# z3lx/waifu2x-tensorrt

Hardware: AMD Instinct MI355X
Metric: upscaled MPix/s, 1080p->4K swin_unet/art fp16 (higher is better)
Workload: dtype f16; 1 GPU; configs[2]: swin_unet/art scale4 noise3 batch4 tile256 fp16, 1920x1080 frame, blend=0.0625 (45 tiles, 12 batches); synthetic-weight graph of that architecture, frame resident in HBM; frames_per_rank=132, parallelism=frame-sharded x1, no collectives; timing barrier over gloo, mode=frames, tiles_per_network_pass=48, tile_groups_per_pass=2

## Files before the change

### waifu2x-tensorrt_amd/csrc/engine.cpp

```cpp
#include <hip/hip_runtime.h>
#include <dlfcn.h>

#include <algorithm>
#include <array>
#include <chrono>
#include <cmath>
#include <cstdio>
#include <cstdlib>
#include <cstring>
#include <deque>
#include <filesystem>
#include <fstream>
#include <map>
#include <sstream>
#include <tuple>

#include "../../include/w2x/img2img.h"
#include "common.h"
#include "fragorder.h"
#include "kernels.h"
#include "liveness.h"
#include "lower.h"
#include "plan.h"
#include "schedule.h"
// ... 133 lines not shown

}

struct Img2Img::Impl {
    MessageCallback messageCallback{};
    ProgressCallback progressCallback{};

    void log(Severity s, const std::string& m) { if (messageCallback) messageCallback(s, m); }
    void log(Severity s, const std::string& m, const std::string& fn, int line) { if (messageCallback) messageCallback(s, "[" + fn + "@" + std::to_string(line) + "] " + m); }
    void log(int current, int total, double speed) { Impl* const to = report_to ? report_to : this; if (to->progressCallback) to->progressCallback(current, total, speed); }
    Impl* report_to = nullptr;

    bool loaded = false;
    int device = -1;
    bool poison = false;
    bool check_general = false;
    bool use_graphs = true;
    Plan plan;
    RenderConfig cfg;
    hipStream_t stream = nullptr;
    hipEvent_t ev0 = nullptr, ev1 = nullptr;
    int (*roctx_push)(const char*) = nullptr; int (*roctx_pop)() = nullptr;
    hipEvent_t ev_shard = nullptr;
    hipEvent_t ev_part[kMaxRenderParts] = {nullptr, nullptr, nullptr, nullptr};
    int pipeline_parts = 3;
    size_t shard_halo_slots = 0;
    int shard_rows = 0, shard_cols = 0;
    hipStream_t gstream[3] = {nullptr, nullptr, nullptr};
    hipEvent_t ev_fork = nullptr, ev_join[3] = {nullptr, nullptr, nullptr};
    int groups = 2;
    std::vector<void*> tensors, blobs;
    std::vector<void*> frag_blobs;
    std::vector<void*> perm_blobs;
    std::vector<int> pool_blocks;
    void* arena_base = nullptr; size_t arena_bytes = 0;
    std::vector<GemmParams> gemm;
    int final_op = -1;
    std::vector<Launch> launches;
    std::vector<std::array<void*, 4>> launch_planes;

    bool deep = false;
    uint8_t* d_frame = nullptr; size_t frame_cap = 0;
    uint8_t* d_out = nullptr; size_t out_cap = 0;
    void* d_slab = nullptr; size_t slab_cap = 0;
    void* d_slab2 = nullptr; size_t slab2_cap = 0;
    hipEvent_t ev_g0[2] = {nullptr, nullptr}, ev_cmp[2] = {nullptr, nullptr};
    bool rolling = false;
    bool rolling_ok = true;
    TileSlot* d_slots = nullptr; size_t slots_cap = 0;
    LiveExt* d_live = nullptr; size_t live_cap = 0, live_stride = 0;
    std::vector<LiveExt> h_live;
    std::map<std::pair<int, int>, std::vector<OpExtent>> live_cache;
    void upload_live(const TileGrid& grid, size_t count, hipStream_t on) {
        const size_t nops = plan.ops.size();
        if (!count || !nops) return;
        if (count > live_stride) {
            ensure(d_live, live_cap, (nops * count + 8) * sizeof(LiveExt));
            live_stride = count;
        }
        const bool all = switches().no_dead_skip || check_general || cfg.tta;
        std::map<std::pair<int, int>, int> tile_at;
        if (!all) for (int t = 0; t < grid.count; ++t) tile_at[{grid.in[t].x, grid.in[t].y}] = t;
        auto extents = [&](int w, int h) -> const std::vector<OpExtent>& {
            auto it = live_cache.find({w, h});
            if (it == live_cache.end()) it = live_cache.emplace(std::make_pair(w, h), dead_skip_extents(plan, w, h, false)).first;
            return it->second;
        };
        const std::vector<OpExtent>& whole = extents(plan.Tout, plan.Tout);
        h_live.resize(nops * count);
        for (size_t st = 0; st < count; ++st) {
            const TileSlot& sl = h_slots[st];
            const std::vector<OpExtent>* e = &whole;
            if (!all && sl.valid && sl.aug == 0) {
                const auto it = tile_at.find({sl.x, sl.y});
                if (it != tile_at.end()) e = &extents(grid.out[it->second].w, grid.out[it->second].h);
            }
            for (size_t i = 0; i < nops; ++i) {
                const OpExtent& x = (*e)[i];
                auto u16 = [](int v) { return (uint16_t)std::min(std::max(v, 0), 65535); };
                h_live[i * count + st] = x.all() ? LiveExt{65535, 0, 65535, 0} : LiveExt{u16(x.x.c), u16(x.x.w), u16(x.y.c), u16(x.y.w)};
            }
        }
        hipAssert(hipMemcpy2DAsync(d_live, live_stride * sizeof(LiveExt), h_live.data(), count * sizeof(LiveExt), count * sizeof(LiveExt), nops, hipMemcpyHostToDevice, on));
    }
    float *d_rampx = nullptr, *d_rampy = nullptr;
    int ovx = 0, ovy = 0;
    float* d_blob_in = nullptr; float* d_blob_out = nullptr;
    uint8_t* d_frame2 = nullptr; size_t frame2_cap = 0;
    uint8_t* d_out2 = nullptr; size_t out2_cap = 0;
    hipStream_t s_up = nullptr, s_dn = nullptr;
    hipEvent_t ev_up[2] = {nullptr, nullptr}, ev_comp[2] = {nullptr, nullptr}, ev_dn[2] = {nullptr, nullptr};
    float* d_canvas = nullptr; size_t canvas_cap = 0;
    struct ResizeTables {
        int inW = 0, inH = 0, outW = 0, outH = 0, filter = 0, edge = kEdgeReplicate;
        int *fx = nullptr, *fy = nullptr; float *wx = nullptr, *wy = nullptr;
        int kx = 0, ky = 0, rows_max = 0;
        int rows_max_above = 0;
    };
    std::deque<ResizeTables> rs_tables;
    struct YuvJob { YuvCoefs in, out; int in_bits = 8, out_bits = 8, key = 0, in_layout = kYuvI420, out_layout = kYuvI420, in_siting = kYuvLeft, out_siting = kYuvLeft; };
    uint8_t* d_bgr = nullptr; size_t bgr_cap = 0;
    uint8_t* d_alpha = nullptr; size_t alpha_cap = 0;
    unsigned* d_minmax = nullptr; unsigned* h_minmax = nullptr;
    hipEvent_t ev_minmax = nullptr;
    struct RgbaJob { int bleed = 0; bool skip = false; size_t alpha_slot0 = 0; bool uniform = false; unsigned value = 255; };
    struct GrayJob { bool deep = false; };
    struct PlanarJob { int in_bits = 8, out_bits = 8; };
    struct ChainJob { const void* src = nullptr; void* dst = nullptr; bool dst_fp32 = false; };
    struct Job {
        enum Kind { BGR, YUV, RGBA, GRAY, PLANAR, PLANAR_RGBA } kind = BGR;
        const ResizeTables* rs = nullptr;
        YuvJob yuv;
        RgbaJob rgba;
        GrayJob gray;
        PlanarJob planar;
        ChainJob chain;
    };
    DitherOptions dither;
    unsigned seq_frame = 0;
    const uint16_t* d_noise = nullptr;
    DitherArgs dither_now() {
        const int mode = (int)dither.mode;
        if (mode == kDitherNone) return DitherArgs();
        if (mode == kDitherBlueNoise && !d_noise) {
            hipError_t e = hipSuccess;
            d_noise = dither_table_device(&e);
            hipAssert(e);
        }
        return dither_args(mode, dither.phase + seq_frame * dither.advance, mode == kDitherBlueNoise ? d_noise : nullptr);
    }
    ResizeLight light = ResizeLight::Gamma;
    LightArgs light_now() const { return light_args((int)light); }
    int edge = kEdgeReplicate;
    bool edge_refuses(const char* who, const char* what) {
        if (edge == kEdgeReplicate) return false;
        log(Severity::error, std::string(what) + " not built under setEdge(" + edge_mode_name(edge) + "): only setEdge(replicate) serves this call.", who, __LINE__);
        return true;
    }
    Job job;
    struct JobScope { Impl* im; ~JobScope() { im->job = Job{}; } };
    static constexpr int kChainStages = 4;
    void* d_chain[kChainStages - 1] = {nullptr, nullptr, nullptr}; size_t chain_cap[kChainStages - 1] = {0, 0, 0};
    hipEvent_t ev_chain_done[kChainStages] = {nullptr, nullptr, nullptr, nullptr}, ev_chain_read[kChainStages - 1] = {nullptr, nullptr, nullptr};
    struct StageTables { TileSlot* d_slots = nullptr; size_t slots_cap = 0; LiveExt* d_live = nullptr; size_t live_cap = 0, live_stride = 0; std::vector<LiveExt> h_live; std::vector<TileSlot> h_slots; };
    StageTables chain_tables[kChainStages];
    void swap_tables(int k) {
        StageTables& t = chain_tables[k];
        std::swap(d_slots, t.d_slots); std::swap(slots_cap, t.slots_cap); std::swap(d_live, t.d_live); std::swap(live_cap, t.live_cap); std::swap(live_stride, t.live_stride);
        h_live.swap(t.h_live); h_slots.swap(t.h_slots);
    }
    void ensure_chain(int k, size_t bytes) {
        if (bytes <= chain_cap[k]) return;
        if (d_chain[k]) hipAssert(hipFree(d_chain[k]));
        d_chain[k] = nullptr; chain_cap[k] = 0;
        hipAssert(hipMalloc(&d_chain[k], bytes));
        chain_cap[k] = bytes;
    }
    std::vector<void*> pinned;
    std::vector<void*> host_allocs;
    std::vector<TileSlot> h_slots;

    bool profiling = false;
    struct Stamp { int kind; hipEvent_t a, b; double flops; int op; };
    std::vector<double> op_ms;
    std::vector<Stamp> stamps;
    void stamp_begin(int kind, double flops, int op = -1) {
        if (!profiling) return;
        Stamp st{kind, nullptr, nullptr, flops, op};
        hipAssert(hipEventCreate(&st.a)); hipAssert(hipEventCreate(&st.b));
        hipAssert(hipEventRecord(st.a, stream));
        stamps.push_back(st);
    }
    void stamp_end() { if (profiling) hipAssert(hipEventRecord(stamps.back().b, stream)); }

    void ensure_copy_streams() {
        if (s_up) return;
        hipAssert(hipStreamCreateWithFlags(&s_up, hipStreamNonBlocking));
        hipAssert(hipStreamCreateWithFlags(&s_dn, hipStreamNonBlocking));
        for (int b = 0; b < 2; ++b) { hipAssert(hipEventCreateWithFlags(&ev_up[b], hipEventDisableTiming)); hipAssert(hipEventCreateWithFlags(&ev_comp[b], hipEventDisableTiming)); hipAssert(hipEventCreateWithFlags(&ev_dn[b], hipEventDisableTiming)); }
    }

    bool one_part_stale = false;
    void one_part_slots() {
        if (!one_part_stale) return;
        const size_t stepCount = pass_slots(last_strip.tile_count);
        fill_slots(last_grid, last_strip.first_tile, last_strip.tile_count, 1, 0, stepCount);
        upload_slots(last_grid, stepCount, stepCount);
        hipAssert(hipStreamSynchronize(stream));
        one_part_stale = false;
    }
    int batch_count(int tiles) const { return w2x::batch_count(tiles, cfg.tta ? 8 : 1, plan.userB); }
    size_t pass_slots(int tiles) const { return w2x::pass_slots(tiles, cfg.tta ? 8 : 1, plan.userB, plan.B); }
    void fill_slots(const TileGrid& grid, int first, int tiles, int valid, size_t at, size_t count) {
        const int steps = cfg.tta ? 8 : 1;
        if (h_slots.size() < at + count) h_slots.resize(at + count);
        for (size_t st = 0; st < count; ++st) {
            const int ti = (int)(st / steps), aug = (int)(st % steps);
            TileSlot sl{0, 0, aug, 0};
            if (ti < tiles) { sl.x = grid.in[first + ti].x; sl.y = grid.in[first + ti].y; sl.valid = valid; }
            h_slots[at + st] = sl;
        }
    }
    void upload_slots(const TileGrid& grid, size_t count, size_t slab_slots) {
        ensure(d_slots, slots_cap, count * sizeof(TileSlot));
        hipAssert(hipMemcpyAsync(d_slots, h_slots.data(), count * sizeof(TileSlot), hipMemcpyHostToDevice, stream));
        upload_live(grid, count, stream);
        ensure(d_slab, slab_cap, slab_slots * plan.Tout * plan.Tout * 4 * plan.elt);
    }
    int last_rows = 0, last_cols = 0, last_batches = 0;
    TileGrid last_grid;
    StripPlan last_strip;
    float last_ms = 0.f;

    static constexpr int kRgbaKey = 64;
    static constexpr int kGrayKey = 65;
    static constexpr int kPlanarKey = 67;
    static constexpr int kPlanarRgbaKey = 72;
    static constexpr int kChainKey = 80;
    using GraphKey = std::tuple<const void*, const void*, const void*, const void*, int, int, int, int>;
    struct PassGraphs { hipGraphExec_t g[4] = {nullptr, nullptr, nullptr, nullptr}; int n = 0; };
    std::map<GraphKey, PassGraphs> graphs;
    std::map<GraphKey, int> graph_seen;
    long graph_replays = 0, eager_passes = 0;
    void drop_graphs() {
        for (auto& kv : graphs) for (int k = 0; k < kv.second.n; ++k) if (kv.second.g[k]) (void)hipGraphExecDestroy(kv.second.g[k]);
        graphs.clear(); graph_seen.clear();
    }

    ~Impl() {
        release();
        for (void* h : host_allocs) if (hipHostFree(h) != hipSuccess) (void)hipGetLastError();
    }

    void release() {
        std::unique_ptr<DeviceGuard> guard;
        if (device >= 0) { try { guard.reset(new DeviceGuard(device)); } catch (...) {} }
        drop_graphs();
        if (arena_base) { (void)hipFree(arena_base); arena_base = nullptr; }
        for (void* p : blobs) if (p) (void)hipFree(p);
        for (void* p : frag_blobs) if (p) (void)hipFree(p);
        frag_blobs.clear();
        for (void* p : perm_blobs) if (p) (void)hipFree(p);
        perm_blobs.clear();
        for (const auto& planes : launch_planes) for (void* p : planes) if (p) (void)hipFree(p);
        launch_planes.clear(); launches.clear();
        tensors.clear(); blobs.clear(); gemm.clear();
        for (void* h : pinned) if (hipHostUnregister(h) != hipSuccess) (void)hipGetLastError();
        pinned.clear();
        for (hipEvent_t* e : {&ev_up[0], &ev_up[1], &ev_comp[0], &ev_comp[1], &ev_dn[0], &ev_dn[1]}) if (*e) { (void)hipEventDestroy(*e); *e = nullptr; }
        if (s_up) { (void)hipStreamDestroy(s_up); s_up = nullptr; }
        if (s_dn) { (void)hipStreamDestroy(s_dn); s_dn = nullptr; }
        frame2_cap = out2_cap = 0;
        for (ResizeTables& t : rs_tables) for (void* q : {(void*)t.fx, (void*)t.fy, (void*)t.wx, (void*)t.wy}) if (q) (void)hipFree(q);
        rs_tables.clear(); job = Job{}; d_noise = nullptr;
        if (d_canvas) { (void)hipFree(d_canvas); d_canvas = nullptr; }
        canvas_cap = 0;
        for (int k = 0; k + 1 < kChainStages; ++k) { if (d_chain[k]) (void)hipFree(d_chain[k]); d_chain[k] = nullptr; chain_cap[k] = 0; if (ev_chain_read[k]) { (void)hipEventDestroy(ev_chain_read[k]); ev_chain_read[k] = nullptr; } }
        for (hipEvent_t& e : ev_chain_done) if (e) { (void)hipEventDestroy(e); e = nullptr; }
        for (StageTables& t : chain_tables) { if (t.d_slots) (void)hipFree(t.d_slots); if (t.d_live) (void)hipFree(t.d_live); t = StageTables{}; }
        report_to = nullptr;
        for (void** q : {(void**)&d_bgr, (void**)&d_alpha, (void**)&d_minmax}) if (*q) { (void)hipFree(*q); *q = nullptr; }
        bgr_cap = alpha_cap = 0;
        if (h_minmax) { if (hipHostFree(h_minmax) != hipSuccess) (void)hipGetLastError(); h_minmax = nullptr; }
        if (ev_minmax) { (void)hipEventDestroy(ev_minmax); ev_minmax = nullptr; }
        for (void** p : {(void**)&d_frame, (void**)&d_out, (void**)&d_frame2, (void**)&d_out2, &d_slab, &d_slab2, (void**)&d_slots, (void**)&d_live, (void**)&d_rampx, (void**)&d_rampy, (void**)&d_blob_in, (void**)&d_blob_out})
            if (*p) { (void)hipFree(*p); *p = nullptr; }
        frame_cap = out_cap = slab_cap = slab2_cap = slots_cap = 0;
        live_cap = live_stride = 0; live_cache.clear();
        shard_rows = shard_cols = 0; shard_halo_slots = 0; rolling = false; one_part_stale = false;
        last_rows = last_cols = last_batches = 0;
        if (ev0) { (void)hipEventDestroy(ev0); ev0 = nullptr; }
        if (ev1) { (void)hipEventDestroy(ev1); ev1 = nullptr; }
        if (ev_shard) { (void)hipEventDestroy(ev_shard); ev_shard = nullptr; }
        for (hipEvent_t& e : ev_part) if (e) { (void)hipEventDestroy(e); e = nullptr; }
        for (hipEvent_t& e : ev_g0) if (e) { (void)hipEventDestroy(e); e = nullptr; }
        for (hipEvent_t& e : ev_cmp) if (e) { (void)hipEventDestroy(e); e = nullptr; }
        if (ev_fork) { (void)hipEventDestroy(ev_fork); ev_fork = nullptr; }
        for (hipEvent_t& e : ev_join) if (e) { (void)hipEventDestroy(e); e = nullptr; }
        for (hipStream_t& st : gstream) if (st) { (void)hipStreamDestroy(st); st = nullptr; }
        if (stream) { (void)hipStreamDestroy(stream); stream = nullptr; }
        loaded = false;
    }

    TView tview(const View& v) const {
        TView t;
        if (v.t < 0) return t;
        const TensorDesc& d = plan.tensors[v.t];
        t.p = tensors[v.t]; t.Hs = d.H; t.Ws = d.W; t.Cs = d.C; t.y0 = v.y0; t.x0 = v.x0;
        return t;
    }

    void upload_planes(const std::vector<uint8_t>& w, int N, int K, void*& dh, void*& dl) {
        std::vector<uint16_t> hi((size_t)N * K), lo((size_t)N * K);
        const float* f = (const float*)w.data();
        auto bf = [](float x) { uint32_t u; memcpy(&u, &x, 4); return (uint16_t)((u + 0x7FFFu + ((u >> 16) & 1u)) >> 16); };
        for (size_t k = 0; k < hi.size(); ++k) {
            const uint16_t h = bf(f[k]);
            const uint32_t hu = (uint32_t)h << 16; float hf; memcpy(&hf, &hu, 4);
            hi[k] = h; lo[k] = bf(f[k] - hf);
        }
        for (int pl = 0; pl < 2; ++pl) {
            const std::vector<uint16_t> fr = frag_major(pl ? lo.data() : hi.data(), N, K);
            void*& d = pl ? dl : dh;
            hipAssert(hipMalloc(&d, fr.size() * 2 + 256));
            hipAssert(hipMemcpy(d, fr.data(), fr.size() * 2, hipMemcpyHostToDevice));
        }
    }

    void upload_plan(Precision prec) {
        const std::vector<Launch> candidates = candidate_launches(plan, prec, check_general);
        place_tensors(layout_arena(plan, candidates));
        upload_weights();
        prepare_gemm_params();
        confirm_launches(candidates);
        hipAssert(hipStreamSynchronize(stream));
    }
    void place_tensors(const ArenaLayout& lay) {
        const int nt = (int)plan.tensors.size();
        const size_t arena = lay.bytes;
        hipAssert(hipMalloc(&arena_base, arena + 1024));
        hipAssert(hipMemsetAsync(arena_base, 0, arena + 1024, stream));
        arena_bytes = arena;
        pool_blocks.assign(nt, 0);
        tensors.assign(nt, nullptr);
        for (int t = 0; t < nt; ++t) tensors[t] = lay.placed[t] ? (uint8_t*)arena_base + lay.off[t] : nullptr;
    }
    void upload_weights() {
        blobs.assign(plan.blobs.size(), nullptr);
        for (size_t i = 0; i < plan.blobs.size(); ++i) {
            const auto& d = plan.blobs[i].data;
            hipAssert(hipMalloc(&blobs[i], d.size() + 256));
            hipAssert(hipMemcpy(blobs[i], d.data(), d.size(), hipMemcpyHostToDevice));
        }
        frag_blobs.assign(plan.blobs.size(), nullptr);
        auto upload_frag = [&](int blob, const std::vector<uint16_t>& f) {
            hipAssert(hipMalloc(&frag_blobs[blob], f.size() * 2 + 256));
            hipAssert(hipMemcpy(frag_blobs[blob], f.data(), f.size() * 2, hipMemcpyHostToDevice));
        };
        auto frag_major_blob = [&](int blob, int N, int K) {
            if (frag_blobs[blob]) return;
            const auto& d = plan.blobs[blob].data;
            if (d.size() != (size_t)N * K * 2) throw std::runtime_error("plan: weight shape");
            upload_frag(blob, frag_major((const uint16_t*)d.data(), N, K));
        };
        auto frag_w2_blob = [&](int blob, int Cc) {
            if (frag_blobs[blob]) return;
            const auto& d = plan.blobs[blob].data;
            if (d.size() != (size_t)Cc * Cc * 4) throw std::runtime_error("plan: mlp weight shape");
            upload_frag(blob, frag_w2((const uint16_t*)d.data(), Cc));
        };
        for (const Op& op : plan.ops)
            if (plan.elt == 2 && op.kind == OP_GEMM && ((op.g.omode == 2 && (op.g.amode == 0 || (op.g.amode == 2 && op.g.kh == 1 && op.g.kw == 1))) || (op.g.amode == 2 && op.g.kh == 2 && op.g.kw == 2 && op.g.stride == 2)) && op.g.K % 32 == 0 && op.g.N % 16 == 0 &&
                plan.blobs[op.g.w].data.size() == (size_t)op.g.N * op.g.K * 2) frag_major_blob(op.g.w, op.g.N, op.g.K);
        perm_blobs.assign(plan.blobs.size(), nullptr);
        for (const Op& op : plan.ops)
            if (plan.elt == 2 && op.kind == OP_GEMM && op.g.amode == 2 && op.g.kh == 3 && op.g.kw == 3 && op.g.stride == 1 && op.g.omode == 0 && op.g.K % 32 == 0 && op.g.N % 64 == 0 &&
                plan.blobs[op.g.w].data.size() == (size_t)op.g.N * op.g.K * 2 && !perm_blobs[op.g.w]) {
                const std::vector<uint16_t> f = frag_conv3b((const uint16_t*)plan.blobs[op.g.w].data.data(), op.g.N, op.g.K);
                hipAssert(hipMalloc(&perm_blobs[op.g.w], f.size() * 2 + 256));
                hipAssert(hipMemcpy(perm_blobs[op.g.w], f.data(), f.size() * 2, hipMemcpyHostToDevice));
            }
        for (const Op& op : plan.ops)
            if (plan.elt == 2 && op.kind == OP_GEMM && op.g.amode == 2 && op.g.kh == 3 && op.g.kw == 3 && op.g.stride == 1 && op.g.omode == 0 && op.g.K == 432 && op.g.N == 96 &&
                plan.tensors[op.g.a.t].C == 48 && !frag_blobs[op.g.w]) {
                const auto& d = plan.blobs[op.g.w].data;
                const int Kw = round_up(op.g.K, 8), Kp = 448;
                if (d.size() != (size_t)op.g.N * Kw * 2) throw std::runtime_error("plan: weight shape");
                std::vector<uint16_t> padded((size_t)op.g.N * Kp, 0);
                for (int n = 0; n < op.g.N; ++n) memcpy(&padded[(size_t)n * Kp], d.data() + (size_t)n * Kw * 2, (size_t)op.g.K * 2);
                upload_frag(op.g.w, frag_major(padded.data(), op.g.N, Kp));
            }
        for (const Op& op : plan.ops)
            if (plan.elt == 2 && op.kind == OP_MLP && mlp_supported(op.m.C)) {
                const int Cm = op.m.C;
                const auto& w1 = plan.blobs[op.m.w1].data; const auto& w2 = plan.blobs[op.m.w2].data;
                if (w1.size() != (size_t)2 * Cm * Cm * 2 || w2.size() != w1.size()) throw std::runtime_error("plan: MLP weight size");
                if (!mlp_frag32(Cm)) {
                    if (!frag_blobs[op.m.w1]) upload_frag(op.m.w1, frag_major((const uint16_t*)w1.data(), 2 * Cm, Cm));
                    if (!frag_blobs[op.m.w2]) upload_frag(op.m.w2, frag_w2((const uint16_t*)w2.data(), Cm));
                    continue;
                }
                if (!frag_blobs[op.m.w1]) upload_frag(op.m.w1, frag32_major((const uint16_t*)w1.data(), 2 * Cm, Cm));
                if (!frag_blobs[op.m.w2]) upload_frag(op.m.w2, frag32_w2((const uint16_t*)w2.data(), Cm));
            }
        for (const Op& op : plan.ops)
            if (plan.elt == 2 && op.kind == OP_SWINATTN) { frag_major_blob(op.sa.wqkv, 3 * op.sa.C, op.sa.C); frag_major_blob(op.sa.wproj, op.sa.C, op.sa.C); }
    }
    void prepare_gemm_params() {
        gemm.assign(plan.ops.size(), GemmParams{}); final_op = -1;
        for (size_t i = 0; i < plan.ops.size(); ++i) {
            const Op& op = plan.ops[i];
            if (op.kind != OP_GEMM) continue;
            const GemmOp& g = op.g;
            GemmParams& p = gemm[i];
            p.a = tview(g.a); p.amode = g.amode; p.kh = g.kh; p.kw = g.kw; p.stride = g.stride;
            p.B = plan.B; p.Mrows = g.Mrows; p.aW = g.aW;
            p.win_table = g.win_table >= 0 ? (const int*)blobs[g.win_table] : nullptr;
            p.K = g.K; p.N = g.N; p.Kw = round_up(g.K, 8);
            p.wt = blobs[g.w]; p.wt_frag = frag_blobs[g.w]; p.wt_perm = perm_blobs[g.w]; p.bias = (const float*)blobs[g.bias];
            p.ln = g.ln; p.csum = g.csum >= 0 ? (const float*)blobs[g.csum] : nullptr;
            p.stats_in = g.stats_in >= 0 ? (const float*)tensors[g.stats_in] : nullptr;
            p.act = g.act; p.alpha = g.alpha; p.has_clip = g.has_clip; p.clip_lo = g.clip_lo; p.clip_hi = g.clip_hi;
            p.res = tview(g.res); p.res2 = tview(g.res2); p.out = tview(g.out);
            p.omode = g.omode; p.r = g.r; p.Cout = g.Cout;
            p.stats_out = g.stats_out >= 0 ? (float*)tensors[g.stats_out] : nullptr; p.ln_eps = g.ln_eps;
            p.pool_out = g.pool_out >= 0 ? (float*)tensors[g.pool_out] : nullptr;
            p.a_scale = g.se_scale >= 0 ? (const float*)tensors[g.se_scale] : nullptr;
            p.res_scale = g.res_scale >= 0 ? (const float*)tensors[g.res_scale] : nullptr;
            if ((p.a_scale || p.res_scale) && plan.elt != 2) throw std::runtime_error("plan: folded gates in an fp32 plan");
            if (g.out.t == plan.out_tensor) final_op = (int)i;
            if (p.ln && (!p.stats_in || !p.csum)) throw std::runtime_error("plan: LayerNorm op without statistics");
            if (p.stats_out && p.Cout != p.out.Cs) throw std::runtime_error("plan: statistics over padded rows");
            if (p.pool_out && p.omode != O_ROWS) throw std::runtime_error("plan: pooling on a scattered output");
            if (p.omode == O_PIXSHUF && p.N != p.r * p.r * p.out.Cs) throw std::runtime_error("plan: pixel-shuffle width mismatch");
            if (p.omode != O_PIXSHUF && p.N != p.out.Cs) throw std::runtime_error("plan: output width mismatch");
            if ((p.amode == A_WIN || p.omode == O_WIN) && !p.win_table) throw std::runtime_error("plan: missing window table");
            if (p.a.Cs != 4 && (p.a.Cs % 8)) throw std::runtime_error("plan: unaligned input channels");
        }
        if (final_op < 0) throw std::runtime_error("plan: the output tensor is not produced by a fused op");
    }
    void confirm_launches(const std::vector<Launch>& candidates) {
        auto head_supported = [&](const GemmParams& g) {
            return g.wt_frag && g.out.Cs == 4 && g.a.y0 == 0 && g.a.x0 == 0 && g.a.Ws == g.aW && (long)g.a.Hs * g.a.Ws == g.Mrows && g.Mrows % 32 == 0 && g.aW >= 32 && pixgemm_supported(g) &&
                   (!g.has_clip || (f16_to_f32(f32_to_f16(g.clip_lo)) == g.clip_lo && f16_to_f32(f32_to_f16(g.clip_hi)) == g.clip_hi));
        };
        launches.clear();
        for (const Launch& L : candidates) {
            const GemmParams& p = gemm[L.last]; const GemmParams& q = gemm[L.first];
            const bool ok = L.kind == L_HEAD ? head_supported(p) : L.kind == L_STEM ? conv48_stem_supported(p, q) || conv3_stem_supported(p, q) : L.kind == L_UP ? conv3_up_supported(p, q) : true;
            if (ok) launches.push_back(L);
            else for (int i = L.first; i <= L.last; ++i) launches.push_back(make_launch(plan, L_OP, i, i));
        }
        launch_planes.assign(launches.size(), {{nullptr, nullptr, nullptr, nullptr}});
        for (size_t k = 0; k < launches.size(); ++k) {
            const Launch& L = launches[k]; std::array<void*, 4>& planes = launch_planes[k];
            if (L.kind == L_MLP32 || L.kind == L_ATTN32) {
                const GemmOp& g1 = plan.ops[L.first].g; const GemmOp& g2 = plan.ops[L.last].g;
                upload_planes(plan.blobs[g1.w].data, g1.N, g1.K, planes[0], planes[1]);
                upload_planes(plan.blobs[g2.w].data, g2.N, g2.K, planes[2], planes[3]);
            }
        }
    }

    int ng_now = 1;
    size_t arena_part() const { return arena_part_bytes(arena_bytes, ng_now); }
    uint8_t* group_ptr(const void* full, int grp) const {
        return full ? (uint8_t*)arena_base + arena_group_offset(arena_bytes, ng_now, grp, (size_t)((const uint8_t*)full - (const uint8_t*)arena_base)) : nullptr;
    }
    void run_network(void* out_override, int live = -1, int grp = -1, hipStream_t s = nullptr, const LiveExt* ext = nullptr) {
        if (!s) s = stream;
        const int cap = grp < 0 ? plan.B : plan.B / ng_now;
        if (live < 0 || live > cap) live = cap;
        auto tp = [&](int t) -> uint8_t* { return t < 0 ? nullptr : grp < 0 ? (uint8_t*)tensors[t] : group_ptr(tensors[t], grp); };
        auto lv = [&](int i) -> const LiveExt* { return ext ? ext + (size_t)i * live_stride : nullptr; };
        auto gp = [&](int i) {
            GemmParams p = gemm[i];
            p.B = live;
            if (grp >= 0) {
                auto shift = [&](auto*& ptr) { ptr = (std::remove_reference_t<decltype(ptr)>)group_ptr(ptr, grp); };
                shift(p.a.p); shift(p.res.p); shift(p.res2.p); shift(p.out.p); shift(p.stats_in); shift(p.stats_out); shift(p.pool_out); shift(p.a_scale); shift(p.res_scale);
            }
            if (i == final_op && out_override) p.out.p = out_override;
            return p;
        };
        for (const Launch& L : launches) try {
            const std::array<void*, 4>& planes = launch_planes[&L - launches.data()];
            const Op& op = plan.ops[L.first];
            struct Range { Impl* e; bool on; ~Range() { if (on) e->roctx_pop(); } } range{this, roctx_push != nullptr};
            if (range.on) roctx_push(launch_label(plan, L).c_str());
            auto issue = [&](auto&& f) { stamp_begin(L.family, L.flops, L.timed); hipAssert(f()); stamp_end(); };
            switch (L.kind) {
                case L_HEAD: {
                    const GemmParams g = gp(L.last);
                    MlpParams p = mlp_params(op, live, tp);
                    p.live = lv(L.last);
                    p.ti_w = g.wt_frag; p.ti_b = g.bias; p.ti_out = g.out.p; p.ti_Hs = g.out.Hs; p.ti_Ws = g.out.Ws; p.ti_Mrows = g.Mrows; p.ti_aW = g.aW;
                    p.ti_clip = g.has_clip; p.ti_lo = g.clip_lo; p.ti_hi = g.clip_hi;
                    issue([&] { return launch_mlp(p, s); });
                    break;
                }
                case L_STEM: case L_UP: {
                    const GemmParams p = gp(L.last), q = gp(L.first);
                    issue([&] { return L.kind == L_UP ? launch_conv3_up(p, q, s) : q.N == 48 ? launch_conv48_stem(p, q, s) : launch_conv3_stem(p, q, s); });
                    break;
                }
                case L_MLP32: {
                    const GemmParams p = gp(L.first), q = gp(L.last);
                    Mlp32Params m;
                    m.x = (const float*)p.a.p; m.y = (float*)q.out.p; m.M = (long)live * p.Mrows; m.C = p.K; m.stats_in = p.stats_in;
                    m.w1h = planes[0]; m.w1l = planes[1]; m.w2h = planes[2]; m.w2l = planes[3];
                    m.b1 = p.bias; m.b2 = q.bias; m.stats_out = q.stats_out; m.eps_out = q.ln_eps;
                    issue([&] { return launch_mlp32(m, s); });
                    break;
                }
                case L_ATTN32: {
                    const GemmParams p = gp(L.first), q = gp(L.last);
                    const AttnOp& a = plan.ops[L.first + 1].at;
                    SwinAttn32Params m;
                    m.x = (const float*)p.a.p; m.y = (float*)q.out.p; m.res = (const float*)q.res.p; m.B = live; m.nwin = a.nwin; m.C = p.K; m.pix_per_item = p.Mrows;
                    m.table_in = p.win_table; m.table_out = q.win_table; m.stats_in = p.stats_in;
                    m.wqkv_h = planes[0]; m.wqkv_l = planes[1]; m.wproj_h = planes[2]; m.wproj_l = planes[3];
                    m.bqkv = p.bias; m.bproj = q.bias; m.scale = a.scale; m.bias = (const float*)blobs[a.bias]; m.maskid = (const int*)blobs[a.maskid];
                    m.stats_out = q.stats_out; m.eps_out = q.ln_eps;
                    issue([&] { return launch_swinattn32(m, s); });
                    break;
                }
                case L_OP: switch (op.kind) {
                    case OP_GEMM: {
                        const GemmParams p = gp(L.first);
                        if (op.g.pool_out >= 0) pool_blocks[op.g.pool_out] = plan.elt == 2 && conv3_supported(p) ? conv3_tiles(p) : 0;
                        issue([&] { return plan.elt == 4 ? launch_gemm_f32(p, s, cfg.precision == Precision::FP32) : pixgemm_supported(p) ? launch_pixgemm(p, s) : conv3_supported(p) ? launch_conv3(p, s) : conv3h_supported(p) ? launch_conv3h(p, s) : conv48_supported(p) ? launch_conv48(p, s) : stem_supported(p) ? launch_stem(p, s) : launch_gemm(p, s); });
                        if (check_general && plan.elt == 2 && (pixgemm_supported(p) || conv3_supported(p) || conv3h_supported(p) || conv48_supported(p) || stem_supported(p))) check_against_general(p, L.first, live);
                        break;
                    }
                    case OP_ATTN: {
                        const AttnOp& a = op.at;
                        AttnParams p;
                        p.qkv = tp(a.qkv); p.out = tp(a.out); p.B = live; p.nwin = a.nwin; p.heads = a.heads; p.hd = a.hd;
                        p.ntok = a.ws * a.ws; p.scale = a.scale; p.bias = blobs[a.bias]; p.maskid = (const int*)blobs[a.maskid];
                        issue([&] { return plan.elt == 4 ? launch_attn_f32(p, s) : launch_attn(p, s); });
                        break;
                    }
                    case OP_SWINATTN: {
                        const SwinAttnOp& a = op.sa;
                        const TensorDesc& d = plan.tensors[a.x];
                        SwinAttnParams p;
                        p.x = tp(a.x); p.y = tp(a.y); p.table = (const int*)blobs[a.table]; p.H = a.H; p.W = a.W; p.ry = a.ry; p.rx = a.rx; p.B = live; p.nwin = a.nwin; p.C = a.C; p.hd = a.hd;
                        p.wqkv = blobs[a.wqkv]; p.bqkv = (const float*)blobs[a.bqkv]; p.scale = a.scale; p.bias32 = (const float*)blobs[a.bias]; p.maskid = (const int*)blobs[a.maskid];
                        p.wproj = blobs[a.wproj]; p.bproj = (const float*)blobs[a.bproj]; p.eps = a.eps;
                        p.wqkv_frag = frag_blobs[a.wqkv]; p.wproj_frag = frag_blobs[a.wproj];
                        p.stats_out = (float*)tp(a.stats_out); p.eps_out = a.eps_out;
                        p.live = lv(L.first);
                        if (d.C != a.C || plan.tensors[a.y].C != a.C || d.H * d.W != a.nwin * a.ws * a.ws) throw std::runtime_error("plan: attention geometry mismatch");
                        issue([&] { return launch_swin_attn(p, s); });
                        break;
                    }
                    case OP_MLP: {
                        MlpParams p = mlp_params(op, live, tp);
                        p.live = lv(L.first);
                        issue([&] { return launch_mlp(p, s); });
                        break;
                    }
                    case OP_SE: {
                        const SeOp& se = op.se;
                        SeParams p;
                        p.pool = (const float*)tp(se.pool); p.scale = (float*)tp(se.scale); p.B = live; p.C = se.C;
                        p.Cs = plan.tensors[se.pool].C; p.Cmid = se.Cmid; p.inv_count = se.inv_count; p.nblocks = pool_blocks[se.pool] > 0 ? pool_blocks[se.pool] : se.nblocks; p.Mrows = se.Mrows;
                        p.w1 = (const float*)blobs[se.w1]; p.b1 = (const float*)blobs[se.b1]; p.w2 = (const float*)blobs[se.w2]; p.b2 = (const float*)blobs[se.b2];
                        issue([&] { return launch_se(p, s); });
                        break;
                    }
                    case OP_SCALE_ADD: {
                        const TensorDesc& d = plan.tensors[op.se.pool];
                        issue([&] { return launch_scale(tp(op.se.pool), (const float*)tp(op.se.scale), live, d.H * d.W, d.C, plan.elt == 4, s); });
                        break;
                    }
                    default: throw std::runtime_error("plan: unknown op kind");
                }
            }
        } catch (const std::exception& e) {
            throw std::runtime_error("op " + launch_label(plan, L) + ": " + e.what());
        }
    }
    template <class TP> MlpParams mlp_params(const Op& op, int live, const TP& tp) const {
        const MlpOp& m = op.m;
        const TensorDesc& d = plan.tensors[m.x];
        MlpParams p;
        p.x = tp(m.x); p.y = tp(m.y); p.M = (long)live * d.H * d.W; p.C = m.C;
        p.w1 = blobs[m.w1]; p.b1 = (const float*)blobs[m.b1]; p.w2 = blobs[m.w2]; p.b2 = (const float*)blobs[m.b2];
        p.w1_frag = frag_blobs[m.w1]; p.w2_frag = frag_blobs[m.w2]; p.frag32 = mlp_frag32(m.C);
        p.eps = m.eps; p.stats_out = (float*)tp(m.stats_out); p.eps_out = m.eps_out;
        p.live_W = d.W; p.live_H = d.H;
        if (d.C != m.C || plan.tensors[m.y].C != m.C) throw std::runtime_error("plan: MLP width mismatch");
        return p;
    }
    void check_against_general(const GemmParams& p, int i, int live) {
        const Op& op = plan.ops[i];
        const TensorDesc& od = plan.tensors[op.g.out.t];
        const size_t n = (size_t)live * od.H * od.W * od.C;
        std::vector<uint16_t> a(n), b(n);
        void* tmp = nullptr;
        hipAssert(hipMalloc(&tmp, n * 2));
        hipAssert(hipStreamSynchronize(stream));
        hipAssert(hipMemcpy(a.data(), p.out.p, n * 2, hipMemcpyDeviceToHost));
        hipAssert(hipMemcpy(tmp, p.out.p, n * 2, hipMemcpyDeviceToDevice));
        GemmParams q = p; q.out.p = tmp; q.pool_out = nullptr;
        hipAssert(launch_gemm(q, stream));
        hipAssert(hipStreamSynchronize(stream));
        hipAssert(hipMemcpy(b.data(), tmp, n * 2, hipMemcpyDeviceToHost));
        hipAssert(hipFree(tmp));
        double md = 0; size_t at = 0, bad = 0;
        for (size_t k = 0; k < n; ++k) { const double d = std::fabs(f16_to_f32(a[k]) - f16_to_f32(b[k])); if (d > 0.01) ++bad; if (d > md) { md = d; at = k; } }
        log(Severity::warn, "pixgemm check op " + std::to_string(i) + " [" + op.name + "]: max|d|=" + std::to_string(md) + " at pixel " + std::to_string(at / od.C) +
            " ch " + std::to_string(at % od.C) + " (x=" + std::to_string(at / od.C % od.W) + ", y=" + std::to_string(at / od.C / od.W % od.H) + "), " + std::to_string(bad) + " of " + std::to_string(n) + " off by > 0.01");
    }

    template <class T> void ensure(T*& p, size_t& cap, size_t bytes) {
        if (bytes <= cap) return;
        drop_graphs();
        if (p) hipAssert(hipFree(p));
        p = nullptr; cap = 0;
        hipAssert(hipMalloc((void**)&p, bytes));
        cap = bytes;
    }

    void run_frame(int rows, int cols, const TileGrid& grid, bool report, const StripPlan& sp, hipEvent_t started = nullptr) {
        if (two_tile_sets()) { rgba_frame(rows, cols, grid, sp, report, started); return; }
        if (started) hipAssert(hipEventRecord(started, stream));
        run_passes(rows, cols, sp.tile_count, 0, report, 0, true);
        finish_frame(rows, cols, grid, sp, stream, nullptr, nullptr);
    }

    bool can_roll(int tile_count) const {
        return rolling_ok && groups == 2 && use_graphs && !profiling && !check_general && !poison && gstream[0] && last_pass_live(tile_count, cfg.tta ? 8 : 1, plan.B) >= 8 && plan.B % 2 == 0;
    }
    void run_rolling_frame(int rows, int cols, const TileGrid& grid, const StripPlan& sp, int which, hipEvent_t out_free) {
        for (int k = 0; k < 2; ++k) {
            if (!ev_g0[k]) hipAssert(hipEventCreateWithFlags(&ev_g0[k], hipEventDisableTiming));
            if (!ev_cmp[k]) hipAssert(hipEventCreateWithFlags(&ev_cmp[k], hipEventDisableTiming));
        }
        struct Swap { Impl* e; void* slab; size_t cap; bool on; ~Swap() { if (on) { std::swap(e->d_slab, e->d_slab2); std::swap(e->slab_cap, e->slab2_cap); } e->rolling = false; } } sw{this, d_slab, slab_cap, which == 1};
        if (which == 1) { std::swap(d_slab, d_slab2); std::swap(slab_cap, slab2_cap); }
        rolling = true;
        hipAssert(hipStreamWaitEvent(stream, ev_cmp[which], 0));
        run_passes(rows, cols, sp.tile_count, 0, false, 0, true);
        hipAssert(hipEventRecord(ev_g0[which], stream));
        hipStream_t s2 = gstream[0];
        hipAssert(hipStreamWaitEvent(s2, ev_g0[which], 0));
        finish_frame(rows, cols, grid, sp, s2, ev_cmp[which], out_free);
    }
    void end_rolling() { hipAssert(hipEventRecord(ev_join[0], gstream[0])); hipAssert(hipStreamWaitEvent(stream, ev_join[0], 0)); }
    void drain_after_error() {
        rolling = false;
        for (hipStream_t st : {s_up, s_dn, gstream[0], stream}) if (st && hipStreamSynchronize(st) != hipSuccess) (void)hipGetLastError();
    }
    template <class Body> bool entry(const char* who, const char* not_ready, const char* failed, const Body& body) try {
        if (!loaded) { log(Severity::error, not_ready, who, __LINE__); return false; }
        DeviceGuard guard(device);
        JobScope job_scope{this};
        return body();
    } catch (const std::exception& e) {
        drain_after_error();
        log(Severity::error, failed + std::string(e.what()) + ".", who, __LINE__);
        return false;
    }

    template <class RunGroup, class RunPass>
    std::string capture_pass(bool per_group, int ngroups, const RunGroup& run_group, const RunPass& run_pass, PassGraphs& pg) {
        std::string why;
        const int ncap = per_group ? ngroups : 1;
        for (int c = 0; c < ncap && why.empty(); ++c) {
            hipStream_t cs = per_group && c ? gstream[c - 1] : stream;
            hipGraph_t graph = nullptr; hipGraphExec_t exec = nullptr;
            hipError_t ge = hipStreamBeginCapture(cs, hipStreamCaptureModeThreadLocal);
            if (ge != hipSuccess) { why = std::string("begin capture: ") + hipGetErrorString(ge); break; }
            try { if (per_group) run_group(c); else run_pass(); } catch (const std::exception& e) { why = std::string("capture: ") + e.what(); }
            ge = hipStreamEndCapture(cs, &graph);
            if (why.empty() && ge != hipSuccess) why = std::string("end capture: ") + hipGetErrorString(ge);
            if (why.empty()) { ge = hipGraphInstantiate(&exec, graph, nullptr, nullptr, 0); if (ge != hipSuccess) why = std::string("instantiation: ") + hipGetErrorString(ge); }
            if (graph) (void)hipGraphDestroy(graph);
            if (why.empty()) pg.g[pg.n++] = exec;
        }
        return why;
    }

    void run_passes(int rows, int cols, int tile_count, size_t slab_slot0, bool report, size_t slots_off, bool fresh, int batch0 = 0, int batch_total = 0, int pass0 = 0, int pass1 = -1) {
        const int B = plan.B, T = plan.T, To = plan.Tout;
        const int steps = cfg.tta ? 8 : 1;
        const int userB = plan.userB, S = B / userB;
        const int batchCount = batch_count(tile_count);
        const int passCount = (int)(pass_slots(tile_count) / B);
        const size_t slot_bytes = (size_t)To * To * 4 * plan.elt;
        if (poison && fresh) {
            hipAssert(hipMemsetAsync(arena_base, 0x7E, arena_bytes, stream));
            hipAssert(hipMemsetAsync(d_slab, 0x7E, slab_cap, stream));
        }
        const bool graphable = use_graphs && !profiling && !check_general;
        for (int bi = pass0; bi < (pass1 < 0 ? passCount : std::min(pass1, passCount)); ++bi) {
            const auto t0 = std::chrono::steady_clock::now();
            const int live = std::max(0, std::min(B, tile_count * steps - bi * B));
            void* const slab_out = (uint8_t*)d_slab + (slab_slot0 + (size_t)bi * B) * slot_bytes;
            GatherParams gp0;
            gp0.frame = d_frame; gp0.rows = rows; gp0.cols = cols; gp0.step = bgr_step(cols, deep); gp0.deep = deep ? 1 : 0;
            gp0.out = tensors[plan.in_tensor]; gp0.slots = d_slots + slots_off + (size_t)bi * B; gp0.B = B; gp0.T = T; gp0.fp32 = plan.elt == 4;
            const int NG = groups;
            struct NgReset { int& r; ~NgReset() { r = 1; } } ng_reset{ng_now};
            ng_now = NG;
            const bool split = NG > 1 && !profiling && !check_general && live >= 4 * NG && B % NG == 0 && (size_t)NG * arena_part() <= arena_bytes + 1024;
            ng_now = 1;
            int first[5] = {0, 0, 0, 0, 0};
            for (int grp = 0; grp < NG; ++grp) first[grp + 1] = first[grp] + live / NG + (grp < live % NG ? 1 : 0);
            if (split) {
                if (!ev_fork) hipAssert(hipEventCreateWithFlags(&ev_fork, hipEventDisableTiming));
                for (int k = 0; k + 1 < NG; ++k) if (!gstream[k]) {
                    hipAssert(hipStreamCreateWithFlags(&gstream[k], hipStreamNonBlocking));
                    hipAssert(hipEventCreateWithFlags(&ev_join[k], hipEventDisableTiming));
                }
            }
            auto group_stream = [&](int grp) { return grp ? gstream[grp - 1] : stream; };
            auto gather_group = [&](int grp, hipStream_t gs) {
                GatherParams gp = gp0;
                gp.out = group_ptr(tensors[plan.in_tensor], grp); gp.slots = gp0.slots + (size_t)first[grp]; gp.B = first[grp + 1] - first[grp];
                gather_tiles(gp, gs);
            };
            const LiveExt* const ext0 = d_live && slots_off + (size_t)(bi + 1) * B <= live_stride ? d_live + slots_off + (size_t)bi * B : nullptr;
            auto network_group = [&](int grp, hipStream_t gs) { run_network((uint8_t*)slab_out + (size_t)first[grp] * slot_bytes, first[grp + 1] - first[grp], grp, gs, ext0 ? ext0 + first[grp] : nullptr); };
            auto fork = [&] { hipAssert(hipEventRecord(ev_fork, stream)); for (int grp = 1; grp < NG; ++grp) hipAssert(hipStreamWaitEvent(gstream[grp - 1], ev_fork, 0)); };
            auto join = [&] { for (int grp = 1; grp < NG; ++grp) { hipAssert(hipEventRecord(ev_join[grp - 1], gstream[grp - 1])); hipAssert(hipStreamWaitEvent(stream, ev_join[grp - 1], 0)); } };
            auto run_pass = [&] {
                if (!split) {
                    stamp_begin(3, 0);
                    gather_tiles(gp0, stream);
                    stamp_end();
                    run_network(slab_out, live, -1, nullptr, ext0);
                    return;
                }
                ng_now = NG;
                for (int grp = 0; grp < NG; ++grp) gather_group(grp, stream);
                fork();
                for (int grp = 0; grp < NG; ++grp) network_group(grp, group_stream(grp));
                join();
                ng_now = 1;
            };
            auto run_group = [&](int grp) { ng_now = NG; gather_group(grp, group_stream(grp)); network_group(grp, group_stream(grp)); ng_now = 1; };
            const bool per_group = split;
            const bool no_join = rolling && split;
            auto run_eager = [&] { if (per_group) { fork(); for (int grp = 0; grp < NG; ++grp) run_group(grp); if (!no_join) join(); } else { if (rolling && gstream[0]) { join(); } run_pass(); } };
            if (!graphable) run_eager();
            else {
                const GraphKey key{pass_source(), d_slots + slots_off + (size_t)bi * B, slab_out, arena_base, rows, cols, live, sample_format()};
                auto replay = [&](const PassGraphs& pg) {
                    if (pg.n == 1) { if (rolling && gstream[0]) join(); hipAssert(hipGraphLaunch(pg.g[0], stream)); return; }
                    fork();
                    for (int grp = 0; grp < pg.n; ++grp) hipAssert(hipGraphLaunch(pg.g[grp], group_stream(grp)));
                    if (!no_join) join();
                };
                auto it = graphs.find(key);
                if (it != graphs.end()) { replay(it->second); ++graph_replays; }
                else if (graph_seen.size() >= 4096 && !graph_seen.count(key)) { graph_seen.clear(); run_eager(); ++eager_passes; }
                else if (graph_seen[key]++ == 0 && !(rolling && !graphs.empty())) { run_eager(); ++eager_passes; }
                else {
                    if (graphs.size() >= 1024) drop_graphs();
                    PassGraphs pg;
                    if (const std::string why = capture_pass(per_group, NG, run_group, run_pass, pg); !why.empty()) {
                        (void)hipGetLastError();
                        for (int c = 0; c < pg.n; ++c) (void)hipGraphExecDestroy(pg.g[c]);
                        use_graphs = false;
                        log(Severity::warn, "hipGraph " + why + " - passes stay on plain launches");
                        run_eager(); ++eager_passes;
                    } else {
                        graphs[key] = pg;
                        replay(pg); ++graph_replays;
                    }
                }
            }
            if (report) {
                const auto t1 = std::chrono::steady_clock::now();
                const double ms = std::chrono::duration<double, std::milli>(t1 - t0).count();
                for (int k = bi * S; k < std::min((bi + 1) * S, batchCount); ++k)
                    log(batch0 + k + 1, batch_total > 0 ? batch_total : batchCount, 1000.0 * S / std::max(ms, 1e-6));
            }
        }
        last_batches = batch0 + batchCount;
    }

    void compose_rect(int rows, int cols, const TileGrid& grid, int x0, int x1, int y0, int y1, long first_tile, hipStream_t on = nullptr) {
        ComposeParams cp = compose_base(rows, cols, grid);
        cp.dst = d_out; cp.dst_step = bgr_step(cp.outW, deep); cp.deep = deep ? 1 : 0;
        cp.x0 = x0; cp.x1 = x1; cp.y0 = y0; cp.y1 = y1; cp.first_tile = first_tile;
        stamp_begin(4, 0);
        hipAssert(launch_compose(cp, on ? on : stream, dither_now()));
        stamp_end();
    }
    ComposeParams compose_base(int rows, int cols, const TileGrid& grid) const {
        const int To = plan.Tout;
        ComposeParams cp;
        cp.tiles = d_slab; cp.fp32 = plan.elt == 4;
        cp.outW = cols * cfg.scaling; cp.outH = rows * cfg.scaling; cp.To = To;
        cp.nx = grid.nx; cp.ny = grid.ny; cp.stride_x = To - grid.outOvX; cp.stride_y = To - grid.outOvY;
        const bool overlapping = cfg.overlapX != 0 || cfg.overlapY != 0;
        cp.ovx = overlapping ? ovx : 0; cp.ovy = overlapping ? ovy : 0;
        cp.ramp_x = d_rampx; cp.ramp_y = d_rampy; cp.tta = cfg.tta ? 1 : 0; cp.tta_bug_compat = cfg.ttaBugCompat ? 1 : 0;
        return cp;
    }
    template <class Params> void resample_base(Params& rp) const {
        const ResizeTables* const rs = job.rs;
        rp.canvas = d_canvas; rp.inW = rs->inW; rp.inH = rs->inH;
        rp.outW = rs->outW; rp.outH = rs->outH;
        rp.fx = rs->fx; rp.wx = rs->wx; rp.kx = rs->kx; rp.fy = rs->fy; rp.wy = rs->wy; rp.ky = rs->ky; rp.rows_max = rs->rows_max;
    }
    static size_t bgr_step(int cols, bool deep16) { return (size_t)cols * 3 * (deep16 ? 2 : 1); }
    static YuvPlanes yuv_layout(uint8_t* base, int rows, int cols, int bits, int layout) {
        const size_t bps = bits > 8 ? 2 : 1;
        const int cw = yuv_chroma_samples(cols, layout), ch = yuv_chroma_rows(rows, layout);
        YuvPlanes f;
        f.rows = rows; f.cols = cols; f.bits = bits; f.layout = layout;
        f.step[0] = ((size_t)cols * bps + 15) / 16 * 16; f.step[1] = f.step[2] = ((size_t)cw * bps + 15) / 16 * 16;
        f.p[0] = base; f.p[1] = base + f.step[0] * rows; f.p[2] = layout == kYuvNV12 ? nullptr : f.p[1] + f.step[1] * ch;
        return f;
    }
    static size_t planar_step(int cols, int bits) { return ((size_t)cols * planar_sample_bytes(bits) + 15) / 16 * 16; }
    static PlanarPlanes planar_layout(uint8_t* base, int rows, int cols, int bits, int n = 3) {
        PlanarPlanes f;
        f.rows = rows; f.cols = cols; f.bits = bits; f.n = n;
        for (int k = 0; k < n; ++k) { f.step[k] = planar_step(cols, bits); f.p[k] = base + (size_t)k * f.step[k] * rows; }
        return f;
    }
    static int planar_key(int bits) { return kPlanarKey + (bits == 8 ? 0 : bits == 10 ? 1 : bits == 12 ? 2 : bits == 16 ? 3 : 4); }
    static int yuv_planes(int layout) { return layout == kYuvNV12 ? 2 : 3; }
    static size_t yuv_bytes(int rows, int cols, int bits, int layout) {
        const YuvPlanes f = yuv_layout(nullptr, rows, cols, bits, layout);
        return f.step[0] * rows + (yuv_planes(layout) - 1) * f.step[1] * yuv_chroma_rows(rows, layout);
    }

    static constexpr int kEdgeKey = 1024;
    int sample_format() const { return frame_format() + kEdgeKey * edge; }
    int frame_format() const {
        if (job.chain.src) return kChainKey;
        switch (job.kind) {
            case Job::YUV: return job.yuv.key;
            case Job::RGBA: return kRgbaKey;
            case Job::GRAY: return kGrayKey + (job.gray.deep ? 1 : 0);
            case Job::PLANAR: return planar_key(job.planar.in_bits);
            case Job::PLANAR_RGBA: return planar_key(job.planar.in_bits) - kPlanarKey + kPlanarRgbaKey;
            default: return deep ? 1 : 0;
        }
    }
    int plane_bits(bool out) const { return job.kind == Job::GRAY ? (job.gray.deep ? 16 : 8) : out ? job.planar.out_bits : job.planar.in_bits; }
    PlanarPlanes frame_planes(uint8_t* base, int rows, int cols, bool out) const { return planar_layout(base, rows, cols, plane_bits(out), job.kind == Job::GRAY ? 1 : 3); }
    const void* pass_source() const { return job.chain.src ? job.chain.src : two_tile_sets() ? (const void*)d_bgr : (const void*)d_frame; }
    bool two_tile_sets() const { return job.kind == Job::RGBA || job.kind == Job::PLANAR_RGBA; }
    RgbaPlanes rgba_planes(uint8_t* base, int rows, int cols, bool out) const {
        const int bits = plane_bits(out);
        RgbaPlanes f;
        f.rows = rows; f.cols = cols; f.bits = bits;
        for (int k = 0; k < 4; ++k) { f.step[k] = planar_step(cols, bits); f.p[k] = base + (size_t)k * f.step[k] * rows; }
        return f;
    }
    size_t bleed_plane_bytes(int rows, int cols) const { return job.kind == Job::PLANAR_RGBA ? planar_step(cols, job.planar.in_bits) * rows : (size_t)rows * cols; }
    unsigned alpha_top() const { return job.kind == Job::PLANAR_RGBA ? alpha_key_top(job.planar.in_bits) : 255u; }
    void launch_bleed(int rows, int cols, int radius) {
        if (job.kind == Job::PLANAR_RGBA) {
            AlphaBleedPlanesParams bp;
            bp.src = rgba_planes(d_frame, rows, cols, false); bp.radius = radius;
            bp.colour_step = bp.alpha_step = planar_step(cols, job.planar.in_bits);
            for (int k = 0; k < 3; ++k) bp.colour[k] = d_bgr + (size_t)k * bp.colour_step * rows;
            bp.alpha = d_alpha; bp.minmax = d_minmax;
            hipAssert(launch_alpha_bleed_planes(bp, stream, edge == kEdgeWrap));
            return;
        }
        AlphaBleedParams bp;
        bp.bgra = d_frame; bp.step = (size_t)cols * 4; bp.rows = rows; bp.cols = cols; bp.radius = radius;
        bp.bgr = d_bgr; bp.bgr_step = (size_t)cols * 3; bp.alpha = d_alpha; bp.alpha_step = (size_t)cols; bp.minmax = d_minmax;
        hipAssert(launch_alpha_bleed(bp, stream, edge == kEdgeWrap));
// ... 270 lines not shown
        if (opt.bleed < 0 || opt.bleed > kBleedMaxRadius) return "Alpha bleed radius " + std::to_string(opt.bleed) + " is not in [0, " + std::to_string(kBleedMaxRadius) + "].";
        return call_grid(c);
    }
    std::string gray_check(const Image* srcs, const Image* dsts, int count, int resizeFilter, const char* who, bool single, FrameCall& c) const {
        const int depth = srcs[0].depth;
        if (single) {
            if ((depth != 8 && depth != 16) || dsts[0].depth != depth) return "Input and output images must both be 8-bit or both 16-bit.";
        } else {
            for (int i = 0; i < count; ++i) if (srcs[i].depth != 8 || dsts[i].depth != 8) return std::string(who) + " takes 8-bit frames (16-bit images go through renderGray()).";
        }
        if (const std::string why = packed_check(srcs, dsts, count, resizeFilter, depth == 16 ? 2 : 1, c); !why.empty()) return why;
        return call_grid(c);
    }
    std::string planar_check(const PlanarImage* srcs, const PlanarImage* dsts, int count, int resizeFilter, FrameCall& c) const {
        const int rows = srcs[0].rows, cols = srcs[0].cols, in_bits = srcs[0].bits, out_bits = dsts[0].bits;
        if (!planar_bits_ok(in_bits) || !planar_bits_ok(out_bits)) return "Planar frames must have 8, 10, 12, 16 or 32 (float) bits.";
        if (rows <= 0 || cols <= 0) return "Input image is empty.";
        if (const std::string why = call_target(resizeFilter, dsts[0], rows, cols, true, c); !why.empty()) return why;
        auto planes_ok = [](const PlanarImage& f) {
            const size_t bps = planar_sample_bytes(f.bits);
            for (int k = 0; k < 3; ++k) if (!f.planes[k] || f.steps[k] < (size_t)f.cols * bps || ((((size_t)f.planes[k]) | f.steps[k]) & (bps - 1)) != 0) return false;
            return true;
        };
        for (int i = 0; i < count; ++i) {
            if (srcs[i].rows != rows || srcs[i].cols != cols || srcs[i].bits != in_bits) return "Input images must be of one size and depth.";
            if (!planes_ok(srcs[i])) return "Input image has a missing plane or an invalid step.";
            if (dsts[i].rows != c.out_rows || dsts[i].cols != c.out_cols) return out_size_text(c);
            if (dsts[i].bits != out_bits) return "Output images must be of one depth.";
            if (!planes_ok(dsts[i])) return "Output image has a missing plane or an invalid step.";
        }
        return call_grid(c);
    }
    std::string planar_rgba_check(const PlanarRgbaImage* srcs, const PlanarRgbaImage* dsts, int count, const RgbaOptions& opt, int resizeFilter, FrameCall& c) const {
        const int rows = srcs[0].rows, cols = srcs[0].cols, in_bits = srcs[0].bits, out_bits = dsts[0].bits;
        if (!planar_bits_ok(in_bits) || !planar_bits_ok(out_bits)) return "Planar frames must have 8, 10, 12, 16 or 32 (float) bits.";
        if (rows <= 0 || cols <= 0) return "Input image is empty.";
        if (const std::string why = call_target(resizeFilter, dsts[0], rows, cols, true, c); !why.empty()) return why;
        for (int i = 0; i < count; ++i) {
            if (srcs[i].rows != rows || srcs[i].cols != cols || srcs[i].bits != in_bits) return "Input images must be of one size and depth.";
            if (!rgba_planes_ok(srcs[i])) return "Input image has a missing plane or an invalid step.";
            if (dsts[i].rows != c.out_rows || dsts[i].cols != c.out_cols) return out_size_text(c);
            if (dsts[i].bits != out_bits) return "Output images must be of one depth.";
            if (!rgba_planes_ok(dsts[i])) return "Output image has a missing plane or an invalid step.";
        }
        if (const std::string why = bleed_problem(opt.bleed, in_bits); !why.empty()) return why;
        return call_grid(c);
    }
    static bool rgba_planes_ok(const PlanarRgbaImage& f) {
        const size_t bps = planar_sample_bytes(f.bits);
        for (int k = 0; k < 4; ++k) if (!f.planes[k] || f.steps[k] < (size_t)f.cols * bps || ((((size_t)f.planes[k]) | f.steps[k]) & (bps - 1)) != 0) return false;
        return true;
    }
    static std::string bleed_problem(int radius, int bits) {
        if (radius < 0 || radius > kBleedMaxRadius) return "Alpha bleed radius " + std::to_string(radius) + " is not in [0, " + std::to_string(kBleedMaxRadius) + "].";
        if (radius > 0 && bits == 32) return "Colour bleed takes integer samples.";
        return "";
    }
    std::string frame_grid(int rows, int cols, TileGrid& grid) const {
        const int s = cfg.scaling;
        grid = calculate_tiles(cols, rows, cols * s, rows * s, plan.T, plan.T, plan.Tout, plan.Tout, s, cfg.overlapX, cfg.overlapY);
        if (grid.count <= 0) return "Tile grid is empty.";
        for (const Rect& r : grid.out) if (r.w <= 0 || r.h <= 0) return "Tile grid does not fit the output (scaling does not match the model).";
        return "";
    }
    void sequence_buffers(size_t in_bytes, size_t out_bytes) {
        ensure_copy_streams();
        ensure(d_frame, frame_cap, in_bytes);   ensure(d_frame2, frame2_cap, in_bytes);
        ensure(d_out, out_cap, out_bytes);      ensure(d_out2, out2_cap, out_bytes);
    }
    void job_resize(int rows, int cols, int out_rows, int out_cols, int resizeFilter) {
        const int s = cfg.scaling;
        job.rs = resize_tables(cols * s, rows * s, out_cols, out_rows, resizeFilter);
        ensure_canvas((size_t)rows * s * cols * s * canvas_planes() * sizeof(float));
    }
    template <class Up, class Down>
    void run_call(const FrameCall& c, int count, bool single, int resizeFilter, const Up& up, const Down& down) {
        const size_t in_bytes = frame_bytes(c.rows, c.cols, false), out_bytes = frame_bytes(c.out_rows, c.out_cols, true);
        if (single) { ensure(d_frame, frame_cap, in_bytes); ensure(d_out, out_cap, out_bytes); }
        else sequence_buffers(in_bytes, out_bytes);
        if (!replayable()) { deep = false; last_rows = last_cols = 0; }
        call_slots(c.rows, c.cols, c.grid, c.sp);
        if (!replayable()) one_part_stale = false;
        if (c.resized) job_resize(c.rows, c.cols, c.out_rows, c.out_cols, resizeFilter);
        if (!single) { last_ms = run_sequence(count, c.rows, c.cols, c.grid, c.sp, up, down) / count; return; }
        up(0, d_frame, stream);
        run_frame(c.rows, c.cols, c.grid, true, c.sp, ev0);
        hipAssert(hipEventRecord(ev1, stream));
        down(0, d_out, stream);
        hipAssert(hipStreamSynchronize(stream));
        hipAssert(hipEventElapsedTime(&last_ms, ev0, ev1));
    }
    void run_packed_call(const FrameCall& c, const Image* srcs, Image* dsts, int count, bool single, int resizeFilter, size_t bpp) {
        const size_t in_step = frame_step(c.cols, false), out_step = frame_step(c.out_cols, true);
        run_call(c, count, single, resizeFilter,
            [&](int i, uint8_t* dev, hipStream_t on) { hipAssert(hipMemcpy2DAsync(dev, in_step, srcs[i].data, srcs[i].step, (size_t)c.cols * bpp, c.rows, hipMemcpyHostToDevice, on)); },
            [&](int i, uint8_t* dev, hipStream_t on) { hipAssert(hipMemcpy2DAsync(dsts[i].data, dsts[i].step, dev, out_step, (size_t)c.out_cols * bpp, c.out_rows, hipMemcpyDeviceToHost, on)); });
    }
    void run_frame_in_parts(const FrameCall& c, const RenderParts& rp, const Image& src, Image& dst) {
        const int rows = c.rows, cols = c.cols, steps = cfg.tta ? 8 : 1;
        const size_t px = deep ? 6 : 3;
        ensure_copy_streams();
        for (int k = 0; k < rp.n; ++k) if (!ev_part[k]) hipAssert(hipEventCreateWithFlags(&ev_part[k], hipEventDisableTiming));
        bool roll = true;
        for (int k = 0; k < rp.n; ++k) roll = roll && can_roll(rp.part[k].tiles);
        struct Unroll { Impl* e; ~Unroll() { e->rolling = false; } } unroll{this};
        if (roll) for (int k = 0; k < 2; ++k) if (!ev_g0[k]) hipAssert(hipEventCreateWithFlags(&ev_g0[k], hipEventDisableTiming));
        for (int k = 0; k < rp.n; ++k) {
            const RenderParts::Part& p = rp.part[k];
            if (k == 1 && rp.x_split < cols) hipAssert(hipStreamWaitEvent(stream, ev_up[0], 0));
            rolling = roll;
            run_passes(rows, cols, p.tiles, (size_t)p.first * steps, true, p.slots_off, k == 0, p.batches_before, rp.batch_total);
            rolling = false;
            if (k == 0 && rp.x_split < cols) {
                hipAssert(hipMemcpy2DAsync(d_frame + (size_t)rp.x_split * px, (size_t)cols * px, src.data + (size_t)rp.x_split * px, src.step, (size_t)(cols - rp.x_split) * px, rows,
                                           hipMemcpyHostToDevice, s_dn));
                hipAssert(hipEventRecord(ev_up[0], s_dn));
            }
            hipStream_t cs = stream;
            if (roll) {
                cs = gstream[0];
                hipAssert(hipEventRecord(ev_g0[k & 1], stream));
                hipAssert(hipStreamWaitEvent(cs, ev_g0[k & 1], 0));
            }
            for (int r = 0; r < p.nrect; ++r) compose_rect(rows, cols, c.grid, p.rect[r].x, p.rect[r].x + p.rect[r].w, p.rect[r].y, p.rect[r].y + p.rect[r].h, 0, cs);
            hipAssert(hipEventRecord(ev_part[k], cs));
            if (k + 1 == rp.n) { if (roll) end_rolling(); hipAssert(hipEventRecord(ev1, stream)); }
        }
        for (int k = 0; k < rp.n; ++k) {
            hipAssert(hipStreamWaitEvent(s_up, ev_part[k], 0));
            for (int r = 0; r < rp.part[k].nrect; ++r) {
                const Rect& rc = rp.part[k].rect[r];
                hipAssert(hipMemcpy2DAsync(dst.data + (size_t)rc.y * dst.step + (size_t)rc.x * px, dst.step, d_out + ((size_t)rc.y * dst.cols + rc.x) * px, (size_t)dst.cols * px,
                                           (size_t)rc.w * px, rc.h, hipMemcpyDeviceToHost, s_up));
            }
        }
        hipAssert(hipStreamSynchronize(s_up));
        hipAssert(hipStreamSynchronize(stream));
    }
    bool rgba_call(const Image* srcs, Image* dsts, int count, const RgbaOptions& opt, int resizeFilter, const char* who, bool single) {
        FrameCall c;
        if (const std::string why = rgba_check(srcs, dsts, count, opt, resizeFilter, c); !why.empty()) { log(Severity::error, why, who, __LINE__); return false; }
        job.kind = Job::RGBA; job.rgba = RgbaJob{opt.bleed, opt.skipUniformAlpha};
        run_packed_call(c, srcs, dsts, count, single, resizeFilter, 4);
        return true;
    }
    void rgba_setup(int rows, int cols, const TileGrid& grid, bool skip) {
        const int steps = cfg.tta ? 8 : 1, N = grid.count;
        const size_t stepTotal = pass_slots(2 * N), colour = (size_t)N * steps;
        ensure_bleed_planes(rows, cols);
        if (skip) {
            if (!h_minmax) hipAssert(hipHostMalloc((void**)&h_minmax, 2 * sizeof(unsigned), hipHostMallocDefault));
            if (!ev_minmax) hipAssert(hipEventCreateWithFlags(&ev_minmax, hipEventDisableTiming));
        }
        fill_slots(grid, 0, N, kSlotColour, 0, colour);
        fill_slots(grid, 0, N, kSlotAlpha, colour, stepTotal - colour);
        upload_slots(grid, stepTotal, stepTotal);
    }
    void rgba_frame(int rows, int cols, const TileGrid& grid, const StripPlan& sp, bool report, hipEvent_t started) {
        RgbaJob& opt = job.rgba;
        const int steps = cfg.tta ? 8 : 1, B = plan.B, S = plan.B / plan.userB, N = grid.count;
        bleed_frame(rows, cols, opt.bleed);
        if (opt.skip) {
            hipAssert(hipMemcpyAsync(h_minmax, d_minmax, 2 * sizeof(unsigned), hipMemcpyDeviceToHost, stream));
            hipAssert(hipEventRecord(ev_minmax, stream));
        }
        if (started) hipAssert(hipEventRecord(started, stream));
// ... 170 lines not shown
        if (dir.empty()) dir = ".";
        std::vector<fs::path> entries;
        for (const auto& entry : fs::directory_iterator(dir)) if (entry.is_regular_file()) entries.push_back(entry.path());
        std::sort(entries.begin(), entries.end());
        for (const auto& path : entries) {
            if (path.filename().string().rfind(engineName, 0) != 0 || path.extension().string() != kEngineExt) continue;
            const std::string configPath = fs::path(path).replace_extension("").string() + ".json";
            if (!fs::exists(configPath)) continue;
            BuildConfig bc; std::string builtOn;
            deserializeConfig(configPath, bc, builtOn);
            if (!isCompatible(config, bc, builtOn, runningOn)) continue;
            if (isOptimized(config, bc)) { enginePath = path.string(); optimized = true; break; }
            if (enginePath.empty()) enginePath = path.string();
        }
        if (enginePath.empty()) throw std::runtime_error("could not satisfy render configuration");
    } catch (const std::exception& e) {
        W2X_LOG(error, "Failed to find engine file for model \"" + modelPath + "\": " + std::string(e.what()) + ".");
        return false;
    }
    std::ifstream file(enginePath, std::ios::binary | std::ios::ate);
    if (!file.is_open()) { W2X_LOG(error, "Failed to open engine file \"" + enginePath + "\"."); return false; }
    std::streamsize fileSize = file.tellg();
    std::vector<char> engineBuffer((size_t)fileSize);
    file.seekg(0, std::ios::beg);
    file.read(engineBuffer.data(), fileSize);

    impl->release();
    impl->device = dev;
    switches_from_env();
    const Switches& sw = switches();
    impl->poison = sw.poison;
    impl->check_general = sw.check_general;
    impl->use_graphs = !sw.no_graph;
    impl->rolling_ok = !sw.no_rolling;
    impl->pipeline_parts = std::min(kMaxRenderParts, std::max(1, sw.render_parts));
    if (const std::string nd = switches_nondefault(); !nd.empty()) W2X_LOG(warn, "Switches off their defaults: " + nd + ".");
    if (sw.roctx && !impl->roctx_push) {
        if (void* h = dlopen("libroctx64.so", RTLD_NOW | RTLD_GLOBAL)) {
            impl->roctx_push = (int (*)(const char*))dlsym(h, "roctxRangePushA");
            impl->roctx_pop = (int (*)())dlsym(h, "roctxRangePop");
            if (!impl->roctx_push || !impl->roctx_pop) impl->roctx_push = nullptr;
        }
        if (!impl->roctx_push) W2X_LOG(warn, "W2X_ROCTX is set but libroctx64.so could not be loaded: no marker ranges.");
    }
    try {
        impl->plan = Plan::deserialize((const uint8_t*)engineBuffer.data(), engineBuffer.size());
    } catch (const std::exception& e) {
        W2X_LOG(error, "Failed to deserialize engine from buffer: " + std::string(e.what()) + ".");
        return false;
    }
    if (!optimized) {
        W2X_LOG(warn, "Engine \"" + enginePath + "\" is compatible with but not optimized for the render configuration; specialising the plan for batch " +
                          std::to_string(config.batchSize) + ", tile " + std::to_string(config.width) + "x" + std::to_string(config.height) + ".");
        try {
            impl->plan = lower_for_shape(modelPath, config.batchSize, config.channels, config.height, config.width, config.precision != Precision::FP16);
        } catch (const std::exception& e) {
            W2X_LOG(error, "Failed to set input tensor shape: " + std::string(e.what()) + ".");
            return false;
        }
    }
    const Plan& plan = impl->plan;
    if ((plan.elt == 4) != (config.precision != Precision::FP16)) {
        W2X_LOG(error, "Failed to deserialize engine from buffer: precision of the plan differs from the engine's configuration.");
        return false;
    }
    if (plan.userB != config.batchSize || plan.B % std::max(plan.userB, 1) || plan.Cin != config.channels || plan.T != config.height || plan.T != config.width) {
        W2X_LOG(error, "Failed to set input tensor shape.");
        return false;
    }
    hipAssert(hipStreamCreateWithFlags(&impl->stream, hipStreamNonBlocking));
    hipAssert(hipEventCreate(&impl->ev0));
    hipAssert(hipEventCreate(&impl->ev1));
    impl->groups = sw.groups;
    impl->ensure_copy_streams();
    if (impl->groups > 1) { hipAssert(hipStreamCreateWithFlags(&impl->gstream[0], hipStreamNonBlocking)); hipAssert(hipEventCreateWithFlags(&impl->ev_join[0], hipEventDisableTiming)); }
    try {
        impl->upload_plan(config.precision);
    } catch (const std::exception& e) {
        W2X_LOG(error, "Failed to allocate resources: " + std::string(e.what()) + ".");
        impl->release();
        return false;
    }
    impl->cfg = config;
    int folds[L_ATTN32 + 1] = {};
    for (const Launch& L : impl->launches) ++folds[L.kind];
    W2X_LOG(info, "Loaded \"" + enginePath + "\": " + std::to_string(plan.ops.size()) + " ops, " + std::to_string(plan.B) + " tiles per pass, activation arena " +
                      std::to_string(impl->arena_bytes >> 20) + " MiB" +
                      (folds[L_STEM] ? ", " + std::to_string(folds[L_STEM]) + " stem folded into the launch of the convolution behind it" : "") +
                      (folds[L_UP] ? ", " + std::to_string(folds[L_UP]) + " transposed convolution folded into the launch of the convolution behind it" : "") +
                      (folds[L_HEAD] ? ", image head folded into the last MLP launch" : "") +
                      (folds[L_ATTN32] + folds[L_MLP32] ? ", " + std::to_string(folds[L_ATTN32]) + " attention and " + std::to_string(folds[L_MLP32]) + " MLP branches as fused fp32-row launches." : "."));
    impl->ovx = (int)std::lround(plan.T * config.scaling * config.overlapX);
    impl->ovy = (int)std::lround(plan.T * config.scaling * config.overlapY);
    if (config.overlapX != 0 || config.overlapY != 0) {
        auto rx = blend_ramp(impl->ovx), ry = blend_ramp(impl->ovy);
        hipAssert(hipMalloc((void**)&impl->d_rampx, std::max<size_t>(rx.size(), 1) * sizeof(float)));
        hipAssert(hipMalloc((void**)&impl->d_rampy, std::max<size_t>(ry.size(), 1) * sizeof(float)));
        hipAssert(hipMemcpy(impl->d_rampx, rx.data(), rx.size() * sizeof(float), hipMemcpyHostToDevice));
        hipAssert(hipMemcpy(impl->d_rampy, ry.data(), ry.size() * sizeof(float), hipMemcpyHostToDevice));
    }
    impl->loaded = true;
    return true;
} catch (const std::exception& e) {
    W2X_LOG(error, "Engine load failed unexpectedly: " + std::string(e.what()) + ".");
    impl->release();
    return false;
}

bool Img2Img::render(const Image& src, Image& dst) { return renderPart(src, dst, 0, 1, "render"); }

bool Img2Img::renderResized(const Image& src, Image& dst, ResizeFilter filter) {
    return renderPart(src, dst, 0, 1, "renderResized", filter_id(filter));
}

bool Img2Img::renderStrip(const Image& src, Image& dst, int part, int parts) {
    if (impl->edge_refuses("renderStrip", "Strips of a frame are")) return false;
    return renderPart(src, dst, part, parts, "renderStrip");
}

bool Img2Img::renderPart(const Image& src, Image& dst, int part, int parts, const char* who, int resizeFilter) {
    return impl->entry(who, kNotLoaded, kRenderFailed, [&] {
    Impl::FrameCall c;
    if (const std::string why = impl->bgr_frame_check(src, dst, part, parts, resizeFilter, c); !why.empty()) { W2X_LOG_AS(who, error, why); return false; }
    const Plan& plan = impl->plan;
    const int rows = c.rows, cols = c.cols, s = impl->cfg.scaling;
    const size_t bps = src.depth / 8;
    hipStream_t stream = impl->stream;
    impl->ensure(impl->d_frame, impl->frame_cap, Impl::bgr_step(cols, bps == 2) * rows);
    impl->ensure(impl->d_out, impl->out_cap, Impl::bgr_step(dst.cols, bps == 2) * dst.rows);
    if (c.resized) impl->job_resize(rows, cols, dst.rows, dst.cols, resizeFilter);
    impl->deep = bps == 2;
    const StripPlan& sp = c.sp;
    if (sp.tile_count == 0) return true;
    const RenderParts rp = render_parts(c.grid, sp, cols, cols * s, rows * s, plan.T, plan.Tout, impl->cfg.tta ? 8 : 1, plan.userB, plan.B,
                                        parts == 1 && !c.resized ? impl->pipeline_parts : 1);
    hipAssert(hipMemcpy2DAsync(impl->d_frame, (size_t)cols * 3 * bps, src.data, src.step, (size_t)rp.x_split * 3 * bps, rows, hipMemcpyHostToDevice, stream));
    for (int k = 0; k < rp.n; ++k) impl->fill_slots(c.grid, sp.first_tile + rp.part[k].first, rp.part[k].tiles, 1, rp.part[k].slots_off, rp.part[k].slots);
    impl->upload_slots(c.grid, rp.slot_total, rp.slab_slots);

    hipAssert(hipEventRecord(impl->ev0, stream));
    if (rp.n == 1) {
        impl->run_frame(rows, cols, c.grid, true, sp);
        hipAssert(hipEventRecord(impl->ev1, stream));
        const int dx0 = c.resized ? 0 : sp.x0, dx1 = c.resized ? dst.cols : sp.x1;
        hipAssert(hipMemcpy2DAsync(dst.data + (size_t)dx0 * 3 * bps, dst.step, impl->d_out + (size_t)dx0 * 3 * bps, (size_t)dst.cols * 3 * bps, (size_t)(dx1 - dx0) * 3 * bps, dst.rows, hipMemcpyDeviceToHost, stream));
        hipAssert(hipStreamSynchronize(stream));
    } else impl->run_frame_in_parts(c, rp, src, dst);
    hipAssert(hipEventElapsedTime(&impl->last_ms, impl->ev0, impl->ev1));
    impl->last_rows = rows; impl->last_cols = cols; impl->last_grid = c.grid; impl->last_strip = sp;
    impl->one_part_stale = rp.n > 1;
    if (c.resized) impl->last_rows = impl->last_cols = 0;
    if (parts == 1 && impl->slab2_cap < impl->slab_cap && impl->can_roll(sp.tile_count)) impl->ensure(impl->d_slab2, impl->slab2_cap, impl->slab_cap);
    return true;
    });
}

struct ShardPeer { const void* slab = nullptr; size_t halo_slots = 0; int device = -1; hipEvent_t ev = nullptr; int first_tile = 0, tile_count = 0; };

static void shard_phase1(Img2Img::Impl& e, const Image& src, const TileGrid& grid, const ShardPlan& sp, bool report) {
    const int rows = src.rows, cols = src.cols, s = e.cfg.scaling, steps = e.cfg.tta ? 8 : 1;
    e.deep = false;
    e.ensure(e.d_frame, e.frame_cap, (size_t)rows * cols * 3);
    e.ensure(e.d_out, e.out_cap, (size_t)rows * s * cols * s * 3);
    hipAssert(hipMemcpy2DAsync(e.d_frame, (size_t)cols * 3, src.data, src.step, (size_t)cols * 3, rows, hipMemcpyHostToDevice, e.stream));
    const size_t stepCount = e.pass_slots(sp.tile_count);
    e.fill_slots(grid, sp.first_tile, sp.tile_count, 1, 0, stepCount);
    e.shard_halo_slots = halo_slots(sp, steps);
    e.upload_slots(grid, stepCount, e.shard_halo_slots + stepCount);
    hipAssert(hipEventRecord(e.ev0, e.stream));
    e.run_passes(rows, cols, sp.tile_count, e.shard_halo_slots, report, 0, true);
    if (!e.ev_shard) hipAssert(hipEventCreateWithFlags(&e.ev_shard, hipEventDisableTiming));
    hipAssert(hipEventRecord(e.ev_shard, e.stream));
}

static void shard_phase2(Img2Img::Impl& e, int k, const std::vector<ShardPlan>& sp, const std::vector<ShardPeer>& peers, const TileGrid& grid, int rows, int cols, Image& dst) {
    const int steps = e.cfg.tta ? 8 : 1, To = e.plan.Tout;
    const size_t px = (size_t)4 * e.plan.elt, slot_bytes = (size_t)To * To * px;
    const bool overlapping = e.cfg.overlapX != 0 || e.cfg.overlapY != 0;
    int waited = -1;
    bool peer2d = true;
    for (int g = sp[k].halo_first; g < sp[k].first_tile && overlapping; ++g) {
        int q = k - 1;
        while (q >= 0 && !(sp[q].tile_count > 0 && g >= sp[q].first_tile && g < sp[q].first_tile + sp[q].tile_count)) --q;
        if (q < 0 || !peers[q].slab) throw std::runtime_error("shard plan: tile " + std::to_string(g) + " has no owner");
        const ShardPeer& o = peers[q];
        if (q != waited) {
            if (o.ev) hipAssert(hipStreamWaitEvent(e.stream, o.ev, 0));
            waited = q;
            peer2d = o.device == e.device;
            if (!peer2d) {
                int can = 0;
                if (o.device >= 0 && hipDeviceCanAccessPeer(&can, e.device, o.device) == hipSuccess && can) {
                    const hipError_t pe = hipDeviceEnablePeerAccess(o.device, 0);
                    peer2d = pe == hipSuccess || pe == hipErrorPeerAccessAlreadyEnabled;
                }
                (void)hipGetLastError();
            }
        }
        for (int a = 0; a < steps; ++a) {
            const uint8_t* from = (const uint8_t*)o.slab + (o.halo_slots + (size_t)(g - sp[q].first_tile) * steps + a) * slot_bytes;
            uint8_t* to = (uint8_t*)e.d_slab + ((size_t)(g - sp[k].halo_first) * steps + a) * slot_bytes;
            if (!peer2d) {
                if (o.device >= 0) hipAssert(hipMemcpyPeerAsync(to, e.device, from, o.device, slot_bytes, e.stream));
                else hipAssert(hipMemcpyAsync(to, from, slot_bytes, hipMemcpyDefault, e.stream));
                continue;
            }
            int bx = std::min(To, grid.outOvX), by = std::min(To, grid.outOvY);
            if (steps > 1) bx = by = std::max(bx, by);
            const size_t pitch = (size_t)To * px;
            auto cols_band = [&](int x0) { if (bx > 0) hipAssert(hipMemcpy2DAsync(to + (size_t)x0 * px, pitch, from + (size_t)x0 * px, pitch, (size_t)bx * px, To, hipMemcpyDeviceToDevice, e.stream)); };
            auto rows_band = [&](int y0) { if (by > 0) hipAssert(hipMemcpyAsync(to + (size_t)y0 * pitch, from + (size_t)y0 * pitch, (size_t)by * pitch, hipMemcpyDeviceToDevice, e.stream)); };
            cols_band(To - bx); rows_band(To - by);
            if (steps > 1) { cols_band(0); rows_band(0); }
        }
    }
    for (int r = 0; r < sp[k].nrect; ++r) {
// ... 693 lines not shown
    impl->upload_and_bleed(bgra, radius);
    hipAssert(hipMemcpy2DAsync(bgr.data, bgr.step, impl->d_bgr, (size_t)cols * 3, (size_t)cols * 3, rows, hipMemcpyDeviceToHost, impl->stream));
    hipAssert(hipStreamSynchronize(impl->stream));
    return true;
    });
}

void* Img2Img::allocHost(size_t bytes) try {
    if (!bytes) return nullptr;
    std::unique_ptr<DeviceGuard> guard;
    if (impl->device >= 0) guard.reset(new DeviceGuard(impl->device));
    void* p = nullptr;
    if (hipHostMalloc(&p, bytes, hipHostMallocDefault) != hipSuccess) { (void)hipGetLastError(); return nullptr; }
    impl->host_allocs.push_back(p);
    return p;
} catch (const std::exception&) {
    return nullptr;
}
void Img2Img::freeHost(void* data) try {
    auto it = std::find(impl->host_allocs.begin(), impl->host_allocs.end(), data);
    if (it == impl->host_allocs.end()) return;
    std::unique_ptr<DeviceGuard> guard;
    if (impl->device >= 0) guard.reset(new DeviceGuard(impl->device));
    if (hipHostFree(data) != hipSuccess) (void)hipGetLastError();
    impl->host_allocs.erase(it);
} catch (const std::exception&) {
}

bool Img2Img::pinHost(void* data, size_t bytes) try {
    if (!data || !bytes) return false;
    if (((size_t)data | bytes) & 4095) { W2X_LOG(warn, "pinHost: only whole pages can be page-locked in place (use allocHost)."); return false; }
    DeviceGuard guard(impl->device);
    if (hipHostRegister(data, bytes, hipHostRegisterDefault) != hipSuccess) { (void)hipGetLastError(); return false; }
    impl->pinned.push_back(data);
    return true;
} catch (const std::exception&) {
    return false;
}
void Img2Img::unpinHost(void* data) try {
    DeviceGuard guard(impl->device);
    auto it = std::find(impl->pinned.begin(), impl->pinned.end(), data);
    if (it == impl->pinned.end()) return;
    if (hipHostUnregister(data) != hipSuccess) (void)hipGetLastError();
    impl->pinned.erase(it);
} catch (const std::exception&) {
}

bool Img2Img::infer(const float* input, float* output) try {
    if (!impl->loaded) { W2X_LOG(error, "Infer called before a successful load."); return false; }
    DeviceGuard guard(impl->device);
    const Plan& plan = impl->plan;
    const size_t in_elems = (size_t)plan.B * 3 * plan.T * plan.T, out_elems = (size_t)plan.B * 3 * plan.Tout * plan.Tout;
    const size_t user_in = (size_t)plan.userB * 3 * plan.T * plan.T, user_out = (size_t)plan.userB * 3 * plan.Tout * plan.Tout;
    hipStream_t stream = impl->stream;
    if (!impl->d_blob_in) {
        hipAssert(hipMalloc((void**)&impl->d_blob_in, in_elems * sizeof(float)));
        hipAssert(hipMalloc((void**)&impl->d_blob_out, out_elems * sizeof(float)));
        hipAssert(hipMemsetAsync(impl->d_blob_in, 0, in_elems * sizeof(float), stream));
    }
    hipAssert(hipMemcpyAsync(impl->d_blob_in, input, user_in * sizeof(float), hipMemcpyHostToDevice, stream));
    hipAssert(launch_blob_to_nhwc(impl->d_blob_in, impl->tensors[plan.in_tensor], plan.B, plan.T, plan.elt == 4, stream));
    impl->run_network(nullptr, plan.userB);
    hipAssert(launch_nhwc_to_blob(impl->tensors[plan.out_tensor], impl->d_blob_out, plan.B, plan.Tout, plan.elt == 4, stream));
    hipAssert(hipMemcpyAsync(output, impl->d_blob_out, user_out * sizeof(float), hipMemcpyDeviceToHost, stream));
    hipAssert(hipStreamSynchronize(stream));
    return true;
} catch (const std::exception& e) {
    W2X_LOG(error, "Engine inference failed unexpectedly: " + std::string(e.what()) + ".");
    return false;
}

int Img2Img::outputTileSize() const { return impl->loaded ? impl->plan.Tout : 0; }
int Img2Img::opTimes(double* out, int cap) const { int n = (int)impl->op_ms.size(); for (int i = 0; i < n && i < cap; ++i) out[i] = impl->op_ms[i]; return n; }
int Img2Img::scaling() const { return impl->loaded ? impl->cfg.scaling : 0; }
int Img2Img::passTiles() const { return impl->loaded ? impl->plan.B : 0; }
double Img2Img::planFlops() const { return impl->loaded ? impl->plan.flops : 0.0; }
float Img2Img::lastRenderMs() const { return impl->last_ms; }

float Img2Img::benchResident(int iters) try {
    if (!impl->loaded || impl->last_rows == 0 || iters <= 0) return -1.f;
    DeviceGuard guard(impl->device);
    hipStream_t stream = impl->stream;
    impl->one_part_slots();
    const bool roll = iters > 1 && impl->can_roll(impl->last_strip.tile_count);
    if (roll) impl->ensure(impl->d_slab2, impl->slab2_cap, impl->slab_cap);
    hipAssert(hipEventRecord(impl->ev0, stream));
    for (int i = 0; i < iters; ++i) {
        if (roll) impl->run_rolling_frame(impl->last_rows, impl->last_cols, impl->last_grid, impl->last_strip, i & 1, nullptr);
        else impl->run_frame(impl->last_rows, impl->last_cols, impl->last_grid, false, impl->last_strip);
    }
    if (roll) impl->end_rolling();
    hipAssert(hipEventRecord(impl->ev1, stream));
    hipAssert(hipStreamSynchronize(stream));
    float ms = 0.f;
    hipAssert(hipEventElapsedTime(&ms, impl->ev0, impl->ev1));
    return ms / iters;
} catch (const std::exception& e) {
    W2X_LOG(error, "Bench failed unexpectedly: " + std::string(e.what()) + ".");
    return -1.f;
}

bool Img2Img::residentOutput(void* dst, size_t bytes) try {
    if (!impl->loaded || impl->last_rows == 0 || !dst) return false;
    const size_t s = (size_t)impl->cfg.scaling, bps = impl->deep ? 2 : 1;
    if (bytes != (size_t)impl->last_rows * s * impl->last_cols * s * 3 * bps) return false;
    DeviceGuard guard(impl->device);
    hipAssert(hipMemcpyAsync(dst, impl->d_out, bytes, hipMemcpyDeviceToHost, impl->stream));
    hipAssert(hipStreamSynchronize(impl->stream));
    return true;
} catch (const std::exception& e) {
    W2X_LOG(error, "Reading the resident output failed unexpectedly: " + std::string(e.what()) + ".");
    return false;
}

bool Img2Img::profileFrame(double* out, int cap) try {
    if (!impl->loaded || impl->last_rows == 0 || cap < 31) return false;
    DeviceGuard guard(impl->device);
    for (int i = 0; i < 31; ++i) out[i] = 0;
    impl->one_part_slots();
    impl->profiling = true; impl->stamps.clear();
    impl->run_frame(impl->last_rows, impl->last_cols, impl->last_grid, false, impl->last_strip);
    impl->profiling = false;
    hipAssert(hipStreamSynchronize(impl->stream));
    impl->op_ms.assign(impl->plan.ops.size(), 0.0);
    for (auto& st : impl->stamps) {
        float ms = 0.f;
        hipAssert(hipEventElapsedTime(&ms, st.a, st.b));
        if (st.op >= 0) impl->op_ms[st.op] += ms;
        out[5 * st.kind] += ms; out[5 * st.kind + 1] += 1; out[5 * st.kind + 2] += st.flops;
    }
    if (!impl->stamps.empty()) { float ms = 0.f; hipAssert(hipEventElapsedTime(&ms, impl->stamps.front().a, impl->stamps.back().b)); out[30] = ms; }
    for (auto& st : impl->stamps) { (void)hipEventDestroy(st.a); (void)hipEventDestroy(st.b); }
    impl->stamps.clear();
    return true;
} catch (const std::exception& e) {
    impl->profiling = false;
    W2X_LOG(error, "Profile failed unexpectedly: " + std::string(e.what()) + ".");
    return false;
}

}
```

### waifu2x-tensorrt_amd/csrc/k_mlp96q.hip

```cpp
#include "transformer_device.h"

#include <algorithm>

#ifndef W2X_MLP_EXP
#define W2X_MLP_EXP 0
#endif
#ifndef W2X_MLP_PREFETCH
#define W2X_MLP_PREFETCH 1
#endif
#ifndef W2X_MLP96_PRIO
#define W2X_MLP96_PRIO 1
#endif
#ifndef W2X_MLP_STAGGER
#define W2X_MLP_STAGGER 0
#endif
#ifndef W2X_MLP_PFCH
#define W2X_MLP_PFCH 5
#endif

namespace w2x {
namespace {

constexpr size_t kMaxBufBytes = 0xFFF00000u;

constexpr int C = 96, RW = 32, NWV = 12, NTHR = NWV * 64;
constexpr int LDX = C + 8, PPR = C / 8, KS = C / 16, NT = C / 32, NCH = 2 * C / 32;
constexpr int NP = RW * PPR / 64;
constexpr int SLAB = RW * LDX * 2;
constexpr int W1F = NCH * KS, W2F = NCH * NT * 2;
constexpr int NF = KS;
static_assert(NF == NT * 2, "one ring serves both products");
constexpr int WBYTES = (W1F + W2F) * 1024;
constexpr int BIAS_OFF = WBYTES + NWV * SLAB;
#ifndef W2X_MLP96_DYN
#define W2X_MLP96_DYN 1
#endif
static_assert(!W2X_MLP96_DYN || W2X_MLP_PREFETCH, "the tile counter is read where the next tile's rows are requested: without the prefetch a wave would stop after its first tile");
constexpr int CTR_OFF = BIAS_OFF + 3 * C * 4;
constexpr int SMEM96Q = CTR_OFF + 16;
static_assert(RW * PPR % 64 == 0, "flat piece count");
static_assert(SMEM96Q <= 160 * 1024, "LDS budget");

template <bool TOIMG>
__global__ __launch_bounds__(NTHR, 3) void mlp96q_kernel(const MlpParams p, int ntiles) {
    extern __shared__ __attribute__((aligned(16))) unsigned char smem[];
    const int tid = threadIdx.x, lane = tid & 63;
    const int wv = __builtin_amdgcn_readfirstlane(tid >> 6);
    const int r32 = lane & 31, h = lane >> 5;
    const _Float16* WL = (const _Float16*)smem + lane * 8;
    _Float16* Xw = (_Float16*)(smem + WBYTES + wv * SLAB);

    {
        const uint4v* w1 = (const uint4v*)p.w1_frag;
        const uint4v* w2 = (const uint4v*)p.w2_frag;
        uint4v* dst = (uint4v*)smem;
        constexpr int N1 = W1F * 64, NALL = (W1F + W2F) * 64;
#pragma unroll
        for (int k = 0; k < NALL / NTHR; ++k) {
            const int i = k * NTHR + tid;
            dst[i] = i < N1 ? w1[i] : w2[i - N1];
        }
        if (tid < 3 * C) ((float*)(smem + BIAS_OFF))[tid] = tid < 2 * C ? p.b1[tid] : p.b2[tid - 2 * C];
        if (tid == 0) *(int*)(smem + CTR_OFF) = 0;
    }
#if W2X_MLP_STAGGER
    for (int k = 0; k < (wv >> 2) * W2X_MLP_STAGGER; ++k) __builtin_amdgcn_s_sleep(127);
#endif
    const float* B1s = (const float*)(smem + BIAS_OFF) + h * 4;
    const float* B2s = B1s + 2 * C;
    __syncthreads();

    half8 wr[NF];
#pragma unroll
    for (int i = 0; i < NF; ++i) wr[i] = *(const half8*)(WL + (size_t)i * 512);
    const int gw = blockIdx.x * NWV + wv, nw = gridDim.x * NWV;
    const unsigned xbytes = (unsigned)(p.M * (C * 2));
    const __amdgpu_buffer_rsrc_t XB = make_rsrc(p.x, xbytes), YB = make_rsrc(p.y, xbytes);
    constexpr unsigned TILE_BYTES = RW * C * 2;
    half8 xr[NP];
#define W2X_FETCH(TILE) { const unsigned vo = (unsigned)((W2X_MLP_EXP & 1) ? ((TILE) & 63) : (TILE)) * TILE_BYTES + lane * 16u;   \
        _Pragma("unroll") for (int k = 0; k < NP; ++k) xr[k] = __builtin_bit_cast(half8, __builtin_amdgcn_raw_buffer_load_b128(XB, vo + k * 1024u, 0, W2X_LD_LAST_AUX)); }
    constexpr bool DYN = W2X_MLP96_DYN && !TOIMG;
    auto tile_live = [&](int tl) -> bool {
        if (!p.live || tl >= ntiles) return true;
        const long r0 = (long)tl * RW, left = p.M - r0;
        return live_rows(p.live, p.live_row0 + r0, left < RW ? (int)left : RW, p.live_W, p.live_H);
    };
    auto grab = [&]() -> int {
        int tl;
        do {
            int t = 0;
            if (lane == 0) t = atomicAdd((int*)(smem + CTR_OFF), 1);
            t = __builtin_amdgcn_readfirstlane(t);
            tl = (blockIdx.x + (t / NWV) * (int)gridDim.x) * NWV + t % NWV;
        } while (!tile_live(tl));
        return tl < ntiles ? tl : ntiles;
    };
    auto stride_from = [&](int tl) -> int {
        while (!tile_live(tl)) tl += nw;
        return tl < ntiles ? tl : ntiles;
    };
    int tile = gw, next_tile = ntiles;
    if constexpr (DYN) tile = grab(); else tile = stride_from(gw);
    if (tile < ntiles) W2X_FETCH(tile)
#if W2X_MLP_PREFETCH
#pragma unroll
    for (int k = 0; k < NP; ++k) __builtin_amdgcn_raw_buffer_store_b128(uint4v{}, YB, 0xFFFFF000u + k * 16u, 0, 0);
#endif
#pragma unroll 1
    for (; tile < ntiles; tile = (DYN || W2X_MLP_PREFETCH) ? next_tile : stride_from(tile + nw)) {
        const long row0 = (long)((W2X_MLP_EXP & 1) ? (tile & 63) : tile) * RW;
        const long nrows = p.M - row0 < RW ? p.M - row0 : RW;
#if !W2X_MLP_PREFETCH
        W2X_FETCH(tile)
#endif
#pragma unroll
        for (int k = 0; k < NP; ++k) {
            const int idx = k * 64 + lane, r = idx / PPR, c = idx - r * PPR;
            *(half8*)(Xw + r * LDX + c * 8) = xr[k];
        }
        W2X_PHASE_FENCE();
#if defined(W2X_MLP96_PRIO) && W2X_MLP96_PRIO == 6
        __builtin_amdgcn_s_setprio(1);
#endif
        half8 xreg[KS];
        {
            half8 raw[KS];
// ... 7 lines not shown
#pragma unroll
            for (int ks = 0; ks < KS; ++ks) xreg[ks] = norm8(raw[ks], rstd, nm);
        }
        float16v acc2[NT];
#pragma unroll
        for (int nt = 0; nt < NT; ++nt)
#pragma unroll
            for (int q = 0; q < 4; ++q) {
                const float4v b = *(const float4v*)(B2s + nt * 32 + q * 8);
#pragma unroll
                for (int j = 0; j < 4; ++j) acc2[nt][4 * q + j] = b[j];
            }
#if defined(W2X_MLP96_PRIO) && (W2X_MLP96_PRIO == 1 || W2X_MLP96_PRIO == 5)
        __builtin_amdgcn_s_setprio(1);
#elif defined(W2X_MLP96_PRIO) && W2X_MLP96_PRIO == 2
        __builtin_amdgcn_s_setprio(0);
#elif defined(W2X_MLP96_PRIO) && W2X_MLP96_PRIO == 4
        __builtin_amdgcn_s_setprio(3);
#endif
#pragma unroll
        for (int ch = 0; ch < NCH; ++ch) {
            float16v acc1;
#pragma unroll
            for (int q = 0; q < 4; ++q) {
                const float4v b = *(const float4v*)(B1s + ch * 32 + q * 8);
#pragma unroll
                for (int j = 0; j < 4; ++j) acc1[4 * q + j] = b[j];
            }
#pragma unroll
            for (int i = 0; i < NF; ++i) {
                if (!(W2X_MLP_EXP & 4)) acc1 = __builtin_amdgcn_mfma_f32_32x32x16_f16(wr[i], xreg[i], acc1, 0, 0, 0);
                else acc1[i] += (float)xreg[i][0] + (float)wr[i][0];
                if (!(W2X_MLP_EXP & 8)) wr[i] = *(const half8*)(WL + (size_t)(W1F + ch * NF + i) * 512);
                W2X_RING_FENCE();
            }
#if W2X_MLP_PREFETCH
            if (ch == W2X_MLP_PFCH) {
                if constexpr (DYN) next_tile = grab(); else next_tile = stride_from(tile + nw);
                W2X_FETCH(next_tile)
                W2X_RING_FENCE();
            }
#endif
            half8 a2[2];
#if defined(W2X_MLP96_PRIO) && W2X_MLP96_PRIO == 3
            __builtin_amdgcn_s_setprio(1);
#elif defined(W2X_MLP96_PRIO) && W2X_MLP96_PRIO == 5
            __builtin_amdgcn_s_setprio(0);
#endif
#pragma unroll
            for (int s2 = 0; s2 < 2; ++s2) {
                if (W2X_MLP_EXP & 2) {
                    a2[s2] = (half8){(_Float16)acc1[8 * s2], (_Float16)acc1[8 * s2 + 1], (_Float16)acc1[8 * s2 + 2], (_Float16)acc1[8 * s2 + 3],
                                     (_Float16)acc1[8 * s2 + 4], (_Float16)acc1[8 * s2 + 5], (_Float16)acc1[8 * s2 + 6], (_Float16)acc1[8 * s2 + 7]};
                    continue;
                }
                const float2v g0 = gelu_fast2((float2v){acc1[8 * s2 + 0], acc1[8 * s2 + 1]});
                const float2v g1 = gelu_fast2((float2v){acc1[8 * s2 + 2], acc1[8 * s2 + 3]});
                const float2v g2 = gelu_fast2((float2v){acc1[8 * s2 + 4], acc1[8 * s2 + 5]});
                const float2v g3 = gelu_fast2((float2v){acc1[8 * s2 + 6], acc1[8 * s2 + 7]});
                a2[s2] = (half8){(_Float16)g0[0], (_Float16)g0[1], (_Float16)g1[0], (_Float16)g1[1],
                                 (_Float16)g2[0], (_Float16)g2[1], (_Float16)g3[0], (_Float16)g3[1]};
            }
#if defined(W2X_MLP96_PRIO) && W2X_MLP96_PRIO == 3
            __builtin_amdgcn_s_setprio(0);
#elif defined(W2X_MLP96_PRIO) && W2X_MLP96_PRIO == 5
            __builtin_amdgcn_s_setprio(1);
#endif
            const int nch = ch + 1 < NCH ? ch + 1 : 0;
#pragma unroll
            for (int i = 0; i < NF; ++i) {
                if (!(W2X_MLP_EXP & 4)) acc2[i >> 1] = __builtin_amdgcn_mfma_f32_32x32x16_f16(wr[i], a2[i & 1], acc2[i >> 1], 0, 0, 0);
                else acc2[i >> 1][i] += (float)a2[i & 1][0] + (float)wr[i][1];
                if (!(W2X_MLP_EXP & 8)) wr[i] = *(const half8*)(WL + (size_t)(nch * NF + i) * 512);
                W2X_RING_FENCE();
            }
        }
#if defined(W2X_MLP96_PRIO) && (W2X_MLP96_PRIO == 1 || W2X_MLP96_PRIO >= 4)
        __builtin_amdgcn_s_setprio(0);
#elif defined(W2X_MLP96_PRIO) && W2X_MLP96_PRIO == 2
        __builtin_amdgcn_s_setprio(1);
#endif
        W2X_PHASE_FENCE();
        half8 wfh[2][3];
        if (TOIMG) {
#pragma unroll
            for (int t = 0; t < 2; ++t)
#pragma unroll
                for (int ks = 0; ks < 3; ++ks) wfh[t][ks] = *(const half8*)((const _Float16*)p.ti_w + lane * 8 + (size_t)(t * 3 + ks) * 512);
            W2X_RING_FENCE();
        }
        half8 xres[NP];
#pragma unroll
        for (int k = 0; k < NP; ++k) {
            const int idx = k * 64 + lane, r = idx / PPR, c = idx - r * PPR;
            xres[k] = *(const half8*)(Xw + r * LDX + c * 8);
        }
        W2X_PHASE_FENCE();
#pragma unroll
        for (int nt = 0; nt < NT; ++nt)
#pragma unroll
            for (int q = 0; q < 4; ++q)
                *(half4*)(Xw + r32 * LDX + nt * 32 + q * 8 + h * 4) = (half4){(_Float16)acc2[nt][4 * q], (_Float16)acc2[nt][4 * q + 1], (_Float16)acc2[nt][4 * q + 2], (_Float16)acc2[nt][4 * q + 3]};
        W2X_PHASE_FENCE();
        const unsigned yo = (unsigned)row0 * (C * 2) + lane * 16u;
#pragma unroll
        for (int k = 0; k < NP; ++k) {
            const int idx = k * 64 + lane, r = idx / PPR, c = idx - r * PPR;
            const half8 o = *(const half8*)(Xw + r * LDX + c * 8) + xres[k];
            if (TOIMG) *(half8*)(Xw + r * LDX + c * 8) = o;
            else if (!(W2X_MLP_EXP & 32)) __builtin_amdgcn_raw_buffer_store_b128(__builtin_bit_cast(uint4v, o), YB, yo + k * 1024u, 0, W2X_ST_AUX);
        }
        if (TOIMG) {
            W2X_PHASE_FENCE();
            const int fr16 = lane & 15, g4 = lane >> 4;
            const _Float16* Wt = (const _Float16*)p.ti_w + lane * 8;
            const int row0i = __builtin_amdgcn_readfirstlane((int)(row0 + p.ti_row0));
            const int bimg = row0i / p.ti_Mrows, ml0 = row0i - bimg * p.ti_Mrows;
            const int oy0 = ml0 / p.ti_aW, ox0 = ml0 - oy0 * p.ti_aW;
            _Float16* __restrict__ Og = (_Float16*)p.ti_out + (size_t)bimg * p.ti_Hs * p.ti_Ws * 4;
            const half2v lo2 = {(_Float16)p.ti_lo, (_Float16)p.ti_lo}, hi2 = {(_Float16)p.ti_hi, (_Float16)p.ti_hi};
#pragma unroll
            for (int th = 0; th < 2; ++th) {
                half8 wf[2][3];
#pragma unroll
                for (int t = 0; t < 2; ++t)
#pragma unroll
                    for (int ks = 0; ks < 3; ++ks) wf[t][ks] = th == 0 ? wfh[t][ks] : *(const half8*)(Wt + (size_t)((2 + t) * 3 + ks) * 512);
                float4v acc[2][2];
#pragma unroll
                for (int t = 0; t < 2; ++t) {
                    const float4v b = *(const float4v*)(p.ti_b + (2 * th + t) * 16 + g4 * 4);
#pragma unroll
                    for (int tt = 0; tt < 2; ++tt) acc[t][tt] = b;
                }
#pragma unroll
                for (int tt = 0; tt < 2; ++tt)
#pragma unroll
                    for (int ks = 0; ks < 3; ++ks) {
                        const half8 xa = *(const half8*)(Xw + (tt * 16 + fr16) * LDX + ks * 32 + g4 * 8);
#pragma unroll
                        for (int t = 0; t < 2; ++t) acc[t][tt] = __builtin_amdgcn_mfma_f32_16x16x32_f16(wf[t][ks], xa, acc[t][tt], 0, 0, 0);
                    }
#pragma unroll
                for (int tt = 0; tt < 2; ++tt) {
                    int ox = ox0 + tt * 16 + fr16, oy = oy0;
                    if (ox >= p.ti_aW) { ox -= p.ti_aW; ++oy; }
                    const bool ok = row0 + tt * 16 + fr16 < p.M;
#pragma unroll
                    for (int t = 0; t < 2; ++t) {
                        half2v v01 = {(_Float16)acc[t][tt][0], (_Float16)acc[t][tt][1]}, v23 = {(_Float16)acc[t][tt][2], (_Float16)acc[t][tt][3]};
                        if (p.ti_clip) {
                            asm("v_pk_max_f16 %0, %1, %2\n\tv_pk_min_f16 %0, %0, %3" : "=&v"(v01) : "v"(v01), "v"(lo2), "v"(hi2));
                            asm("v_pk_max_f16 %0, %1, %2\n\tv_pk_min_f16 %0, %0, %3" : "=&v"(v23) : "v"(v23), "v"(lo2), "v"(hi2));
                        }
                        const half4 px = {v01[0], v01[1], v23[0], v23[1]};
                        if (ok) *(half4*)(Og + ((size_t)(oy * 4 + 2 * th + t) * p.ti_Ws + ox * 4 + g4) * 4) = px;
                    }
                }
            }
        }
        if (!TOIMG && p.stats_out) {
#pragma unroll
            for (int k = 0; k < NP; ++k) {
                const int idx = k * 64 + lane, r = idx / PPR, c = idx - r * PPR;
                *(half8*)(Xw + r * LDX + c * 8) = *(const half8*)(Xw + r * LDX + c * 8) + xres[k];
            }
        }
        W2X_PHASE_FENCE();
        if (!TOIMG && p.stats_out && lane < nrows) {
            float s = 0.f, q = 0.f;
#pragma unroll
            for (int c = 0; c < PPR; ++c) sum_sq8_acc(*(const half8*)(Xw + lane * LDX + c * 8), s, q);
            const float mean = s * (1.f / C);
            p.stats_out[2 * (row0 + lane)] = mean;
            p.stats_out[2 * (row0 + lane) + 1] = __builtin_amdgcn_rsqf(fmaxf(q * (1.f / C) - mean * mean, 0.f) + p.eps_out);
        }
        W2X_PHASE_FENCE();
    }
#undef W2X_FETCH
}

}

bool mlp96q_supported(const MlpParams& p) { return p.C == C && p.w1_frag && p.w2_frag && p.frag32 && (!p.ti_w || (p.ti_b && p.ti_out && !p.stats_out && p.ti_Mrows > 0 && p.ti_Mrows % RW == 0 && p.ti_aW >= RW && p.M < 0x7FFFFFFFl &&
                                                                 (!p.ti_clip || ((float)(_Float16)p.ti_lo == p.ti_lo && (float)(_Float16)p.ti_hi == p.ti_hi)))); }

hipError_t launch_mlp96q(const MlpParams& p, hipStream_t s) {
    static unsigned lds_ok = 0;
    static unsigned lds_ok_t = 0;
    if (hipError_t e = p.ti_w ? ensure_dynamic_lds((const void*)mlp96q_kernel<true>, SMEM96Q, lds_ok_t) : ensure_dynamic_lds((const void*)mlp96q_kernel<false>, SMEM96Q, lds_ok); e != hipSuccess) return e;
    static int cus[32] = {0};
    int dev = 0;
    if (hipError_t e = hipGetDevice(&dev); e != hipSuccess) return e;
    int ncu = __atomic_load_n(&cus[dev & 31], __ATOMIC_RELAXED);
    if (ncu == 0) {
        if (hipError_t e = hipDeviceGetAttribute(&ncu, hipDeviceAttributeMultiprocessorCount, dev); e != hipSuccess) return e;
        __atomic_store_n(&cus[dev & 31], ncu, __ATOMIC_RELAXED);
    }
    const long max_tiles = std::min<long>((long)(kMaxBufBytes / (RW * C * 2)), 0xFFFFFFFFl / (RW * C * 2) - (long)ncu * NWV);
    return for_mlp_runs(p, max_tiles * RW, [&](const MlpParams& q) {
        const long ntiles = (q.M + RW - 1) / RW;
        const int grid = (int)std::min<long>((ntiles + NWV - 1) / NWV, ncu);
        if ((ntiles + (long)grid * NWV) * (long)(RW * C * 2) > 0xFFFFFFFFl) return hipErrorInvalidValue;
        if (p.ti_w) hipLaunchKernelGGL(mlp96q_kernel<true>, dim3(grid), dim3(NTHR), SMEM96Q, s, q, (int)ntiles);
        else hipLaunchKernelGGL(mlp96q_kernel<false>, dim3(grid), dim3(NTHR), SMEM96Q, s, q, (int)ntiles);
        return hipGetLastError();
    });
}

}
```

### waifu2x-tensorrt_amd/csrc/k_prepost.hip

```cpp
#include "kernels.h"
#include "prepost_device.h"
#include <type_traits>

namespace w2x {
namespace {

template <typename P, int E = kEdgeReplicate>
__global__ __launch_bounds__(256) void gather_kernel(const GatherParams p) {
    const int T = p.T;
    const long total = (long)p.B * T * T;
    const float inv255 = (float)(1.0 / 255.0), inv65535 = (float)(1.0 / 65535.0);
    for (long i = (long)blockIdx.x * blockDim.x + threadIdx.x; i < total; i += (long)gridDim.x * blockDim.x) {
        int b = (int)(i / ((long)T * T));
        int rem = (int)(i - (long)b * T * T);
        int y = rem / T, x = rem - y * T;
        TileSlot sl = p.slots[b];
        P v = make_px<P>(0.f, 0.f, 0.f);
        if (sl.valid) {
            int sy, sx;
            aug_src(sl.aug, T - 1, y, x, sy, sx);
            int fy = edge_src<E>(sl.y + sy, p.rows);
            int fx = edge_src<E>(sl.x + sx, p.cols);
            if (!p.deep) {
                const uint8_t* px = p.frame + (size_t)fy * p.step + (size_t)fx * 3;
                v = make_px<P>((float)px[2] * inv255, (float)px[1] * inv255, (float)px[0] * inv255);
            } else {
                const uint16_t* px = (const uint16_t*)(p.frame + (size_t)fy * p.step) + (size_t)fx * 3;
                v = make_px<P>((float)px[2] * inv65535, (float)px[1] * inv65535, (float)px[0] * inv65535);
            }
        }
        *((P*)p.out + i) = v;
    }
}

template <typename P, int M>
__device__ __forceinline__ unsigned compose_pixel(const ComposeParams& p, const P* tiles, int X, int Y, const DitherArgs& dz) {
    float a0, a1, a2;
    compose_pixel_sums<P>(p, tiles, X, Y, a0, a1, a2);
    return quantize_bgr_at<M>(a0, a1, a2, dz, X, Y);
}
template <typename Launch> hipError_t for_dither(const DitherArgs& d, Launch launch) {
    if (d.mode == kDitherOrdered) return launch(std::integral_constant<int, kDitherOrdered>());
    if (d.mode == kDitherBlueNoise && d.table) return launch(std::integral_constant<int, kDitherBlueNoise>());
    return hipErrorInvalidValue;
}

typedef _Float16 half8 __attribute__((ext_vector_type(8)));

template <typename P, int M = kDitherNone, typename... D>
__global__ __launch_bounds__(kComposeThreads) void compose_kernel(const ComposeParams p, const D... dzs) {
    static_assert(dither_pack_ok<M, D...>, "kDitherNone: no argument; else one DitherArgs");
    const DitherArgs& dz = dither_of(dzs...);
    constexpr bool kHalf = sizeof(P) == 8;
    const int x1 = p.x1 > 0 ? p.x1 : p.outW, sw = x1 - p.x0;
    const int gw = (sw + 3) >> 2;
    const int xg = blockIdx.x * kComposeThreads + threadIdx.x;
    if (xg >= gw) return;
    const P* tiles = (const P*)p.tiles;
    const int To = p.To, n = To - 1;
    const int X = p.x0 + 4 * xg;
    const int np = min(4, x1 - X);
    int a0 = X - To + 1; a0 = a0 <= 0 ? 0 : (a0 + p.stride_x - 1) / p.stride_x;
    int b0 = X + 3 - To + 1; b0 = b0 <= 0 ? 0 : (b0 + p.stride_x - 1) / p.stride_x;
    const int a1 = min(p.nx - 1, X / p.stride_x), b1 = min(p.nx - 1, (X + 3) / p.stride_x);
    const bool fast_col = kHalf && np == 4 && !p.tta && !p.deep && a0 == b0 && a1 == b1;
    const int Y0 = p.y0 + blockIdx.y * kComposeRows, Y1 = min(p.y1 > 0 ? p.y1 : p.outH, Y0 + kComposeRows);
    for (int Y = Y0; Y < Y1; ++Y) {
        uint8_t* d = p.dst + (size_t)Y * p.dst_step + (size_t)X * 3;
        unsigned px[4] = {0u, 0u, 0u, 0u};
        if (p.deep) {
            uint16_t* d16 = (uint16_t*)(p.dst + (size_t)Y * p.dst_step) + (size_t)X * 3;
            for (int k = 0; k < np; ++k) {
                float r, g, b;
                compose_pixel_sums<P>(p, tiles, X + k, Y, r, g, b);
                if constexpr (M == kDitherNone) {
                    d16[3 * k] = (uint16_t)min(max(__float2int_rn(b * 65535.f), 0), 65535);
                    d16[3 * k + 1] = (uint16_t)min(max(__float2int_rn(g * 65535.f), 0), 65535);
                    d16[3 * k + 2] = (uint16_t)min(max(__float2int_rn(r * 65535.f), 0), 65535);
                } else {
                    d16[3 * k] = (uint16_t)quant_code<M>(b * 65535.f, 65535, dz, 2, X + k, Y);
                    d16[3 * k + 1] = (uint16_t)quant_code<M>(g * 65535.f, 65535, dz, 1, X + k, Y);
                    d16[3 * k + 2] = (uint16_t)quant_code<M>(r * 65535.f, 65535, dz, 0, X + k, Y);
                }
            }
            continue;
        }
        const bool fast = fast_col && (((size_t)d) & 3) == 0;
        if (fast) {
            int j0 = Y - To + 1; j0 = j0 <= 0 ? 0 : (j0 + p.stride_y - 1) / p.stride_y;
            const int j1 = min(p.ny - 1, Y / p.stride_y);
            float acc[4][3] = {};
            for (int ti = a0; ti <= a1; ++ti) {
                const int ox = ti * p.stride_x, lx = X - ox;
                const int rw = ox + To > p.outW ? p.outW - ox : To;
                for (int tj = j0; tj <= j1; ++tj) {
                    const int oy = tj * p.stride_y, ly = Y - oy;
                    const int rh = oy + To > p.outH ? p.outH - oy : To;
                    const long tile = (long)ti * p.ny + tj - p.first_tile;
                    const half4* tp = (const half4*)p.tiles + tile * (long)To * To + (long)ly * To + lx;
                    half4 h[4];
                    if ((((size_t)tp) & 15) == 0) { const half8 u0 = *(const half8*)tp, u1 = *(const half8*)(tp + 2);
                        h[0] = (half4){u0[0], u0[1], u0[2], u0[3]}; h[1] = (half4){u0[4], u0[5], u0[6], u0[7]}; h[2] = (half4){u1[0], u1[1], u1[2], u1[3]}; h[3] = (half4){u1[4], u1[5], u1[6], u1[7]}; }
                    else { h[0] = tp[0]; h[1] = tp[1]; h[2] = tp[2]; h[3] = tp[3]; }
                    const bool wl = ox > 0, wt = oy > 0 && ly < p.ovy, wr = ox + rw < p.outW, wb = oy + rh < p.outH && n - ly < p.ovy;
                    const float fy_t = wt ? p.ramp_y[ly] : 1.f, fy_b = wb ? p.ramp_y[n - ly] : 1.f;
#pragma unroll
                    for (int k = 0; k < 4; ++k) {
                        float v0 = (float)h[k][0], v1 = (float)h[k][1], v2 = (float)h[k][2];
                        if (p.ovx || p.ovy) {
                            const int lk = lx + k;
                            if (wl && lk < p.ovx) { float w = p.ramp_x[lk]; v0 *= w; v1 *= w; v2 *= w; }
                            if (wt) { v0 *= fy_t; v1 *= fy_t; v2 *= fy_t; }
                            if (wr && n - lk < p.ovx) { float w = p.ramp_x[n - lk]; v0 *= w; v1 *= w; v2 *= w; }
                            if (wb) { v0 *= fy_b; v1 *= fy_b; v2 *= fy_b; }
                        }
                        acc[k][0] += v0; acc[k][1] += v1; acc[k][2] += v2;
                    }
                }
            }
#pragma unroll
            for (int k = 0; k < 4; ++k) px[k] = quantize_bgr_at<M>(acc[k][0], acc[k][1], acc[k][2], dz, X + k, Y);
            unsigned* dw = (unsigned*)d;
            dw[0] = px[0] | px[1] << 24;
            dw[1] = px[1] >> 8 | px[2] << 16;
            dw[2] = px[2] >> 16 | px[3] << 8;
        } else {
            for (int k = 0; k < np; ++k) {
                const unsigned v = compose_pixel<P, M>(p, tiles, X + k, Y, dz);
                d[3 * k] = (uint8_t)v; d[3 * k + 1] = (uint8_t)(v >> 8); d[3 * k + 2] = (uint8_t)(v >> 16);
            }
        }
    }
}

template <typename P, typename... L>
__global__ __launch_bounds__(256) void compose_canvas_kernel(const ComposeParams p, float* canvas, const L... ls) {
    static_assert(dither_pack_ok<kDitherNone, L...>, "no argument, or one LightArgs");
    constexpr bool kLin = light_on<L...>;
    const LightArgs& lz = light_of(ls...);
    const int x1 = p.x1 > 0 ? p.x1 : p.outW, y1 = p.y1 > 0 ? p.y1 : p.outH;
    const int X = p.x0 + blockIdx.x * 256 + threadIdx.x;
    if (X >= x1) return;
    const size_t plane = (size_t)p.outW * p.outH;
    for (int Y = p.y0 + blockIdx.y; Y < y1; Y += gridDim.y) {
        float r, g, b;
        compose_pixel_sums<P>(p, (const P*)p.tiles, X, Y, r, g, b);
        const size_t i = (size_t)Y * p.outW + X;
        canvas[i] = light_canvas<kLin>(lz, r); canvas[plane + i] = light_canvas<kLin>(lz, g); canvas[2 * plane + i] = light_canvas<kLin>(lz, b);
    }
}

__device__ __forceinline__ float yuv_sample(const YuvPlanes& f, int pl, int y, int x) {
    const uint8_t* row = f.p[pl] + (size_t)y * f.step[pl];
    return f.bits > 8 ? (float)((const uint16_t*)row)[x] : (float)row[x];
}

template <int L>
__device__ __forceinline__ float yuv_luma(const YuvPlanes& f, int y, int x) {
    if constexpr (L != kYuvNV12) return yuv_sample(f, 0, y, x);
    const uint8_t* row = f.p[0] + (size_t)y * f.step[0];
    return f.bits > 8 ? (float)(((const uint16_t*)row)[x] >> 6) : (float)row[x];
}
template <int L>
__device__ __forceinline__ float yuv_chroma(const YuvPlanes& f, int pl, int y, int x) {
    if constexpr (L != kYuvNV12) return yuv_sample(f, pl, y, x);
    const uint8_t* row = f.p[1] + (size_t)y * f.step[1];
    const int i = 2 * x + pl - 1;
    return f.bits > 8 ? (float)(((const uint16_t*)row)[i] >> 6) : (float)row[i];
}

template <bool kCentred>
__device__ __forceinline__ void yuv_axis_taps(int n, int cn, int& i0, int& i1, float& w0, float& w1) {
    const int k = n >> 1;
    const bool odd = n & 1;
    if constexpr (kCentred) {
        i0 = odd ? k : max(k - 1, 0); i1 = odd ? min(k + 1, cn - 1) : k;
        w0 = odd ? 0.75f : 0.25f; w1 = odd ? 0.25f : 0.75f;
    } else {
        i0 = k; i1 = odd ? min(k + 1, cn - 1) : k;
        w0 = 0.5f; w1 = 0.5f;
    }
}
template <typename P, int L, int S = kYuvLeft>
__global__ __launch_bounds__(256) void gather_yuv_kernel(const GatherYuvParams p) {
    static_assert(S == kYuvLeft || L == kYuvI420 || L == kYuvNV12 || (L == kYuvI422 && S == kYuvCenter), "a siting the layout does not tell from kYuvLeft");
    const int T = p.T;
    const long total = (long)p.B * T * T;
    const int rows = p.src.rows, cols = p.src.cols, ch = (rows + 1) >> 1, cw = (cols + 1) >> 1;
    const YuvCoefs& k = p.k;
    for (long i = (long)blockIdx.x * blockDim.x + threadIdx.x; i < total; i += (long)gridDim.x * blockDim.x) {
        int b = (int)(i / ((long)T * T));
        int rem = (int)(i - (long)b * T * T);
        int y = rem / T, x = rem - y * T;
        TileSlot sl = p.slots[b];
        P v = make_px<P>(0.f, 0.f, 0.f);
        if (sl.valid) {
            int sy, sx;
            aug_src(sl.aug, T - 1, y, x, sy, sx);
            const int fy = min(max(sl.y + sy, 0), rows - 1), fx = min(max(sl.x + sx, 0), cols - 1);
            float u, w;
            if constexpr (S != kYuvLeft) {
                int c0, c1, r0 = fy, r1 = fy;
                float wc0, wc1, w0 = 0.5f, w1 = 0.5f;
                yuv_axis_taps<yuv_cols_centred(S)>(fx, cw, c0, c1, wc0, wc1);
                if constexpr (L != kYuvI422) yuv_axis_taps<yuv_rows_centred(S)>(fy, ch, r0, r1, w0, w1);
                u = w0 * (wc0 * yuv_chroma<L>(p.src, 1, r0, c0) + wc1 * yuv_chroma<L>(p.src, 1, r0, c1)) + w1 * (wc0 * yuv_chroma<L>(p.src, 1, r1, c0) + wc1 * yuv_chroma<L>(p.src, 1, r1, c1));
                w = w0 * (wc0 * yuv_chroma<L>(p.src, 2, r0, c0) + wc1 * yuv_chroma<L>(p.src, 2, r0, c1)) + w1 * (wc0 * yuv_chroma<L>(p.src, 2, r1, c0) + wc1 * yuv_chroma<L>(p.src, 2, r1, c1));
            } else if constexpr (L == kYuvI444) {
                u = yuv_chroma<L>(p.src, 1, fy, fx); w = yuv_chroma<L>(p.src, 2, fy, fx);
            } else if constexpr (L == kYuvI422) {
                const int cj = fx >> 1, c1 = (fx & 1) ? min(cj + 1, cw - 1) : cj;
                u = 0.5f * (yuv_chroma<L>(p.src, 1, fy, cj) + yuv_chroma<L>(p.src, 1, fy, c1));
                w = 0.5f * (yuv_chroma<L>(p.src, 2, fy, cj) + yuv_chroma<L>(p.src, 2, fy, c1));
            } else {
                const int ck = fy >> 1, cj = fx >> 1;
// ... 293 lines not shown
    const int pc = Cs / 8;
    const long total = (long)B * HW * pc;
    for (long i = (long)blockIdx.x * blockDim.x + threadIdx.x; i < total; i += (long)gridDim.x * blockDim.x) {
        int cp = (int)(i % pc);
        long pix = i / pc;
        int b = (int)(pix / HW);
        *((half8*)x + i) = gate::gate8(*((half8*)x + i), scale + b * Cs + cp * 8);
    }
}

__global__ __launch_bounds__(256) void scale32_kernel(float* x, const float* scale, int B, long HW, int Cs) {
    const int pc = Cs / 4;
    const long total = (long)B * HW * pc;
    for (long i = (long)blockIdx.x * blockDim.x + threadIdx.x; i < total; i += (long)gridDim.x * blockDim.x) {
        const int cp = (int)(i % pc);
        const int b = (int)(i / pc / HW);
        float4v v = *((float4v*)x + i);
        const float* sc = scale + b * Cs + cp * 4;
#pragma unroll
        for (int e = 0; e < 4; ++e) v[e] *= sc[e];
        *((float4v*)x + i) = v;
    }
}

template <typename P>
__global__ __launch_bounds__(256) void blob_to_nhwc_kernel(const float* nchw, P* out, int B, int T) {
    const long total = (long)B * T * T;
    for (long i = (long)blockIdx.x * blockDim.x + threadIdx.x; i < total; i += (long)gridDim.x * blockDim.x) {
        int b = (int)(i / ((long)T * T));
        long rem = i - (long)b * T * T;
        const float* s = nchw + (long)b * 3 * T * T + rem;
        out[i] = make_px<P>(s[0], s[(long)T * T], s[2L * T * T]);
    }
}

template <typename P>
__global__ __launch_bounds__(256) void nhwc_to_blob_kernel(const P* in, float* nchw, int B, int T) {
    const long total = (long)B * T * T;
    for (long i = (long)blockIdx.x * blockDim.x + threadIdx.x; i < total; i += (long)gridDim.x * blockDim.x) {
        int b = (int)(i / ((long)T * T));
        long rem = i - (long)b * T * T;
        const P v = in[i];
        float* d = nchw + (long)b * 3 * T * T + rem;
        d[0] = (float)v[0]; d[(long)T * T] = (float)v[1]; d[2L * T * T] = (float)v[2];
    }
}

inline unsigned grid_for(long total) { long g = (total + 255) / 256; return (unsigned)(g > 8192 ? 8192 : (g < 1 ? 1 : g)); }

}

template <int E>
static hipError_t launch_gather_as(const GatherParams& p, dim3 grid, hipStream_t s) {
    if (p.fp32) hipLaunchKernelGGL((gather_kernel<float4v, E>), grid, dim3(256), 0, s, p);
    else hipLaunchKernelGGL((gather_kernel<half4, E>), grid, dim3(256), 0, s, p);
    return hipGetLastError();
}
hipError_t launch_gather(const GatherParams& p, hipStream_t s, int edge) {
    const dim3 grid(grid_for((long)p.B * p.T * p.T));
    switch (edge) {
        case kEdgeReplicate: return launch_gather_as<kEdgeReplicate>(p, grid, s);
        case kEdgeWrap: return launch_gather_as<kEdgeWrap>(p, grid, s);
        case kEdgeMirror: return launch_gather_as<kEdgeMirror>(p, grid, s);
    }
    return hipErrorInvalidValue;
}
hipError_t launch_compose(const ComposeParams& p, hipStream_t s, const DitherArgs& d) {
    if (!dither_args_ok(d)) return hipErrorInvalidValue;
    const int gw = (((p.x1 > 0 ? p.x1 : p.outW) - p.x0) + 3) / 4;
    if (gw <= 0 || p.outH <= 0) return hipSuccess;
    const int nrows = (p.y1 > 0 ? p.y1 : p.outH) - p.y0;
    if (nrows <= 0) return hipSuccess;
    const dim3 grid((unsigned)((gw + kComposeThreads - 1) / kComposeThreads), (unsigned)((nrows + kComposeRows - 1) / kComposeRows));
    if (d.mode != kDitherNone) return for_dither(d, [&](auto m) {
        constexpr int M = decltype(m)::value;
        if (p.fp32) hipLaunchKernelGGL((compose_kernel<float4v, M, DitherArgs>), grid, dim3(kComposeThreads), 0, s, p, d);
        else hipLaunchKernelGGL((compose_kernel<half4, M, DitherArgs>), grid, dim3(kComposeThreads), 0, s, p, d);
        return hipGetLastError();
    });
    if (p.fp32) hipLaunchKernelGGL(compose_kernel<float4v>, grid, dim3(kComposeThreads), 0, s, p);
    else hipLaunchKernelGGL(compose_kernel<half4>, grid, dim3(kComposeThreads), 0, s, p);
    return hipGetLastError();
}
hipError_t launch_compose_canvas(const ComposeParams& p, float* canvas, hipStream_t s, const LightArgs& l) {
    const int w = (p.x1 > 0 ? p.x1 : p.outW) - p.x0, h = (p.y1 > 0 ? p.y1 : p.outH) - p.y0;
    if (w <= 0 || h <= 0) return hipSuccess;
    if (!light_args_ok(l)) return hipErrorInvalidValue;
    const dim3 grid((unsigned)((w + 255) / 256), (unsigned)(h < 65535 ? h : 65535));
    if (l.mode != kLightGamma) {
        if (p.fp32) hipLaunchKernelGGL((compose_canvas_kernel<float4v, LightArgs>), grid, dim3(256), 0, s, p, canvas, l);
        else hipLaunchKernelGGL((compose_canvas_kernel<half4, LightArgs>), grid, dim3(256), 0, s, p, canvas, l);
        return hipGetLastError();
    }
    if (p.fp32) hipLaunchKernelGGL(compose_canvas_kernel<float4v>, grid, dim3(256), 0, s, p, canvas);
    else hipLaunchKernelGGL(compose_canvas_kernel<half4>, grid, dim3(256), 0, s, p, canvas);
    return hipGetLastError();
}
template <int L, int S = kYuvLeft>
static void launch_gather_yuv_as(const GatherYuvParams& p, dim3 grid, hipStream_t s) {
    if (p.fp32) hipLaunchKernelGGL((gather_yuv_kernel<float4v, L, S>), grid, dim3(256), 0, s, p);
    else hipLaunchKernelGGL((gather_yuv_kernel<half4, L, S>), grid, dim3(256), 0, s, p);
}
static int yuv_effective_siting(int layout, int siting) {
    if (siting < kYuvLeft || siting > kYuvTopLeft) return -1;
    if (layout == kYuvI444 || (layout == kYuvI422 && siting == kYuvTopLeft)) return kYuvLeft;
    return siting;
}
hipError_t launch_gather_yuv(const GatherYuvParams& p, hipStream_t s) {
    const dim3 grid(grid_for((long)p.B * p.T * p.T));
    switch (yuv_effective_siting(p.src.layout, p.src.siting)) {
        case kYuvLeft:
            switch (p.src.layout) {
                case kYuvI420: launch_gather_yuv_as<kYuvI420>(p, grid, s); break;
                case kYuvI422: launch_gather_yuv_as<kYuvI422>(p, grid, s); break;
                case kYuvI444: launch_gather_yuv_as<kYuvI444>(p, grid, s); break;
                case kYuvNV12: launch_gather_yuv_as<kYuvNV12>(p, grid, s); break;
                default: return hipErrorInvalidValue;
            }
            break;
        case kYuvCenter:
            switch (p.src.layout) {
                case kYuvI420: launch_gather_yuv_as<kYuvI420, kYuvCenter>(p, grid, s); break;
                case kYuvI422: launch_gather_yuv_as<kYuvI422, kYuvCenter>(p, grid, s); break;
                case kYuvNV12: launch_gather_yuv_as<kYuvNV12, kYuvCenter>(p, grid, s); break;
                default: return hipErrorInvalidValue;
            }
            break;
        case kYuvTopLeft:
            switch (p.src.layout) {
                case kYuvI420: launch_gather_yuv_as<kYuvI420, kYuvTopLeft>(p, grid, s); break;
                case kYuvNV12: launch_gather_yuv_as<kYuvNV12, kYuvTopLeft>(p, grid, s); break;
                default: return hipErrorInvalidValue;
            }
            break;
        default: return hipErrorInvalidValue;
    }
    return hipGetLastError();
}
template <int L, int S, int M, typename... D>
static void launch_compose_yuv_as(const ComposeYuvParams& p, dim3 grid, hipStream_t s, const D&... dz) {
    if (p.c.fp32) hipLaunchKernelGGL((compose_yuv_kernel<float4v, L, S, M, D...>), grid, dim3(kYuvThreads), 0, s, p, dz...);
    else hipLaunchKernelGGL((compose_yuv_kernel<half4, L, S, M, D...>), grid, dim3(kYuvThreads), 0, s, p, dz...);
}
template <int M, typename... D>
static hipError_t launch_compose_yuv_mode(const ComposeYuvParams& p, hipStream_t s, const D&... dz) {
    if (p.c.outW <= 0 || p.c.outH <= 0) return hipSuccess;
    const int siting = yuv_effective_siting(p.dst.layout, p.dst.siting);
    if (siting < 0) return hipErrorInvalidValue;
    if (p.dst.layout == kYuvI444) {
        const int gw = (p.c.outW + 3) / 4;
        const dim3 grid((unsigned)((gw + kComposeThreads - 1) / kComposeThreads), (unsigned)((p.c.outH + kComposeRows - 1) / kComposeRows));
        if (p.c.fp32) hipLaunchKernelGGL((compose_yuv444_kernel<float4v, M, D...>), grid, dim3(kComposeThreads), 0, s, p, dz...);
        else hipLaunchKernelGGL((compose_yuv444_kernel<half4, M, D...>), grid, dim3(kComposeThreads), 0, s, p, dz...);
        return hipGetLastError();
    }
    const int cw = (p.c.outW + 1) / 2, ch = yuv_chroma_rows(p.c.outH, p.dst.layout);
    const int runs = (cw + kYuvSites - 1) / kYuvSites;
    const dim3 grid((unsigned)((runs + kYuvThreads - 1) / kYuvThreads), (unsigned)(ch < 65535 ? ch : 65535));
    if (siting == kYuvTopLeft) {
        const int bands = (ch + kYuvBand - 1) / kYuvBand;
        if (bands > 65535) return hipErrorInvalidValue;
        const dim3 bgrid(grid.x, (unsigned)bands);
        switch (p.dst.layout) {
            case kYuvI420: launch_compose_yuv_as<kYuvI420, kYuvTopLeft, M>(p, bgrid, s, dz...); break;
            case kYuvNV12: launch_compose_yuv_as<kYuvNV12, kYuvTopLeft, M>(p, bgrid, s, dz...); break;
            default: return hipErrorInvalidValue;
// ... 51 lines not shown
```

### waifu2x-tensorrt_amd/csrc/kernels.h

```cpp
#pragma once
#include <hip/hip_runtime.h>

#include "support.h"
#include "switches.h"
#include "dither.h"
#include "light.h"
#include "edge.h"
#include <cstdint>

namespace w2x {

constexpr int kGemmBM = 128;

inline hipError_t ensure_dynamic_lds(const void* fn, int bytes, unsigned& done_mask) {
    int dev = 0;
    hipError_t e = hipGetDevice(&dev);
    if (e != hipSuccess) return e;
    const unsigned bit = 1u << (dev & 31);
    if (__atomic_load_n(&done_mask, __ATOMIC_ACQUIRE) & bit) return hipSuccess;
    e = hipFuncSetAttribute(fn, hipFuncAttributeMaxDynamicSharedMemorySize, bytes);
    if (e == hipSuccess) __atomic_fetch_or(&done_mask, bit, __ATOMIC_RELEASE);
    return e;
}

// ... 14 lines not shown
#endif

struct LiveExt { uint16_t cx, wx, cy, wy; };
#ifdef __HIPCC__
__device__ __forceinline__ LiveExt live_ext_load(const LiveExt* t, int slot) {
    typedef const unsigned long long __attribute__((address_space(4)))* cptr;
    const unsigned long long v = ((cptr)(unsigned long long)t)[slot];
    return LiveExt{(uint16_t)v, (uint16_t)(v >> 16), (uint16_t)(v >> 32), (uint16_t)(v >> 48)};
}
__device__ __forceinline__ bool live_token(const LiveExt e, int x, int y, int W, int H) { return (x < e.cx || x >= W - e.wx) && (y < e.cy || y >= H - e.wy); }
__device__ __forceinline__ bool live_rows(const LiveExt* t, long r0, int n, int W, int H) {
    const int HW = W * H;
    if (n > HW) return true;
    const int img = (int)(r0 / HW);
    int r = (int)(r0 - (long)img * HW);
    LiveExt e = live_ext_load(t, img);
    for (int left = n; left > 0;) {
        if (r >= HW) { r -= HW; e = live_ext_load(t, img + 1); }
        const int y = r / W, x0 = r - y * W, x1 = x0 + left < W ? x0 + left : W;
        if ((y < e.cy || y >= H - e.wy) && (x0 < e.cx || x1 > W - e.wx)) return true;
        left -= x1 - x0; r += x1 - x0;
    }
    return false;
}
#endif

struct TView {
    void* p = nullptr;
    int Hs = 0, Ws = 0, Cs = 0;
    int y0 = 0, x0 = 0;
};

struct GemmParams {
    TView a;
    int amode = 0, kh = 1, kw = 1, stride = 1;
    int B = 0, Mrows = 0, aW = 0;
    const int* win_table = nullptr;
    int K = 0, N = 0, Kw = 0;
    const void* wt = nullptr;
    const void* wt_frag = nullptr;
    const void* wt_perm = nullptr;
    const float* bias = nullptr;
    const float* csum = nullptr;
    const float* stats_in = nullptr;
    int ln = 0;
    int act = 0; float alpha = 0.f;
    int has_clip = 0; float clip_lo = 0.f, clip_hi = 0.f;
    const float* a_scale = nullptr;
    const float* res_scale = nullptr;
    TView res, res2;
    TView out;
    int omode = 0, r = 1, Cout = 0;
    float* stats_out = nullptr; float ln_eps = 1e-5f;
    float* pool_out = nullptr;
};

struct AttnParams {
    const void* qkv = nullptr; void* out = nullptr;
    int B = 0, nwin = 0, heads = 0, hd = 0, ntok = 0;
    float scale = 1.f;
    const void* bias = nullptr;
    const int* maskid = nullptr;
};

struct MlpParams {
    const void* x = nullptr; void* y = nullptr;
    long M = 0; int C = 0;
    const void* w1 = nullptr;
    const float* b1 = nullptr;
    const void* w2 = nullptr;
    const float* b2 = nullptr;
    float eps = 1e-5f;
    float* stats_out = nullptr; float eps_out = 1e-5f;
    const void* w1_frag = nullptr; const void* w2_frag = nullptr;
    bool frag32 = false;
    const void* ti_w = nullptr;
    const float* ti_b = nullptr;
    void* ti_out = nullptr; int ti_Hs = 0, ti_Ws = 0, ti_Mrows = 0, ti_aW = 0;
    int ti_clip = 0; float ti_lo = 0.f, ti_hi = 0.f;
    long ti_row0 = 0;
    const LiveExt* live = nullptr; int live_W = 0, live_H = 0;
    long live_row0 = 0;
};

struct SwinAttnParams {
    const void* x = nullptr; void* y = nullptr;
    const int* table = nullptr;
    int H = 0, W = 0, ry = -1, rx = -1;
    int B = 0, nwin = 0, C = 0, hd = 0;
    const void* wqkv = nullptr;
    const float* bqkv = nullptr;
    float scale = 1.f;
    const float* bias32 = nullptr;
    const int* maskid = nullptr;
    const void* wproj = nullptr;
    const float* bproj = nullptr;
    float eps = 1e-5f;
    float* stats_out = nullptr; float eps_out = 1e-5f;
    const void* wqkv_frag = nullptr; const void* wproj_frag = nullptr;
    const LiveExt* live = nullptr;
};

struct SeParams {
    const float* pool = nullptr; float* scale = nullptr;
    int B = 0, C = 0, Cs = 0, Cmid = 0; float inv_count = 0.f;
    int nblocks = 0, Mrows = 0;
    const float *w1 = nullptr, *b1 = nullptr, *w2 = nullptr, *b2 = nullptr;
};

struct TileSlot { int x, y, aug, valid; };

struct GatherParams {
    const uint8_t* frame = nullptr; int rows = 0, cols = 0; size_t step = 0;
    int deep = 0;
    void* out = nullptr;
    int fp32 = 0;
    const TileSlot* slots = nullptr;
    int B = 0, T = 0;
};

struct ComposeParams {
    const void* tiles = nullptr;
    int fp32 = 0;
    uint8_t* dst = nullptr; size_t dst_step = 0;
    int deep = 0;
    int outW = 0, outH = 0;
    int To = 0;
    int nx = 0, ny = 0;
    int stride_x = 0, stride_y = 0;
    int ovx = 0, ovy = 0;
    const float* ramp_x = nullptr;
    const float* ramp_y = nullptr;
    int tta = 0;
    int tta_bug_compat = 0;
    int x0 = 0, x1 = 0; long first_tile = 0;
    int y0 = 0, y1 = 0;
};

hipError_t launch_gemm(const GemmParams& p, hipStream_t s);
bool pixgemm_supported(const GemmParams& p);
hipError_t launch_pixgemm(const GemmParams& p, hipStream_t s);
int pixgemm_rows_per_workgroup(const GemmParams& p);
bool conv3_supported(const GemmParams& p);
bool stem_supported(const GemmParams& p);
hipError_t launch_stem(const GemmParams& p, hipStream_t s);
hipError_t launch_conv3(const GemmParams& p, hipStream_t s);
bool conv3h_supported(const GemmParams& p);
hipError_t launch_conv3h(const GemmParams& p, hipStream_t s);
bool conv48_supported(const GemmParams& p);
hipError_t launch_conv48(const GemmParams& p, hipStream_t s);
bool conv48_stem_supported(const GemmParams& p, const GemmParams& ps);
hipError_t launch_conv48_stem(const GemmParams& p, const GemmParams& ps, hipStream_t s);
bool conv3_stem_supported(const GemmParams& p, const GemmParams& ps);
hipError_t launch_conv3_stem(const GemmParams& p, const GemmParams& ps, hipStream_t s);
bool conv3_up_supported(const GemmParams& p, const GemmParams& q);
hipError_t launch_conv3_up(const GemmParams& p, const GemmParams& q, hipStream_t s);
int conv3_tiles(const GemmParams& p);
hipError_t launch_attn(const AttnParams& p, hipStream_t s);
hipError_t launch_gemm_f32(const GemmParams& p, hipStream_t s, bool exact);
hipError_t launch_attn_f32(const AttnParams& p, hipStream_t s);
struct Mlp32Params {
    const float* x = nullptr; float* y = nullptr;
    long M = 0; int C = 0;
    const float* stats_in = nullptr;
    const void *w1h = nullptr, *w1l = nullptr, *w2h = nullptr, *w2l = nullptr;
    const float *b1 = nullptr, *b2 = nullptr;
// ... 267 lines not shown
```

### waifu2x-tensorrt_amd/csrc/support.cpp

```cpp
#include "support.h"

namespace w2x {

bool swin_attn_supported(int C, int heads, int hd, int ws) {
    return ws == 6 && heads * hd == C && ((C == 96 && hd == 16) || (C == 192 && hd == 32));
}
bool mlp_supported(int C) { return C == 96 || C == 192; }
bool mlp32_supported(int C) { return C == 96 || C == 192; }
bool swinattn32_supported(int C, int heads, int hd, int ntok) { return heads == 6 && ntok == 36 && ((C == 96 && hd == 16) || (C == 192 && hd == 32)); }
bool gemm_row_stats_supported(int N) { return N == 32 || N == 48 || N == 64 || N == 96 || N == 128 || N == 192; }
bool attn_supported(int hd, int ntok) {
    if (ntok != 36 && ntok != 64) return false;
    return hd == 8 || hd == 16 || hd == 24 || hd == 32 || hd == 48 || hd == 64;
}

}

#include <algorithm>
#include <cstdlib>
#include <cstring>

#include "switches.h"

namespace w2x {

namespace {
struct Field { const char* name; int Switches::*i; bool Switches::*b; const char* env; int lo, hi; };
const Field kFields[] = {
    {"superbatch", &Switches::superbatch, nullptr, "W2X_SUPERBATCH", 0, 4096},
    {"groups", &Switches::groups, nullptr, "W2X_GROUPS", 1, 4},
    {"render_parts", &Switches::render_parts, nullptr, "W2X_RENDER_PARTS", 1, 4},
    {"no_graph", nullptr, &Switches::no_graph, "W2X_NO_GRAPH", 0, 1},
    {"no_rolling", nullptr, &Switches::no_rolling, "W2X_NO_ROLLING", 0, 1},
    {"poison", nullptr, &Switches::poison, "W2X_POISON", 0, 1},
    {"check_general", nullptr, &Switches::check_general, "W2X_CHECK_GENERAL", 0, 1},
    {"roctx", nullptr, &Switches::roctx, "W2X_ROCTX", 0, 1},
    {"no_fuse", nullptr, &Switches::no_fuse, nullptr, 0, 1},
    {"no_fuse_attn", nullptr, &Switches::no_fuse_attn, nullptr, 0, 1},
    {"no_se_fold", nullptr, &Switches::no_se_fold, nullptr, 0, 1},
    {"no_fuse_head", nullptr, &Switches::no_fuse_head, nullptr, 0, 1},
    {"no_fuse_stem", nullptr, &Switches::no_fuse_stem, nullptr, 0, 1},
    {"no_fuse_up", nullptr, &Switches::no_fuse_up, nullptr, 0, 1},
    {"no_conv3h_walk", nullptr, &Switches::no_conv3h_walk, nullptr, 0, 1},
    {"no_pixgemm", nullptr, &Switches::no_pixgemm, nullptr, 0, 1},
    {"no_conv3", nullptr, &Switches::no_conv3, nullptr, 0, 1},
    {"no_conv3h", nullptr, &Switches::no_conv3h, nullptr, 0, 1},
    {"no_conv48", nullptr, &Switches::no_conv48, nullptr, 0, 1},
    {"no_stem", nullptr, &Switches::no_stem, nullptr, 0, 1},
    {"attn_valu", nullptr, &Switches::attn_valu, nullptr, 0, 1},
    {"no_dead_skip", nullptr, &Switches::no_dead_skip, nullptr, 0, 1},
};
void assign(Switches& s, const Field& f, long v) {
    v = std::min<long>(f.hi, std::max<long>(f.lo, v));
    if (f.i) s.*(f.i) = (int)v; else s.*(f.b) = v != 0;
}
}

Switches& switches() { static Switches s; return s; }

void switches_from_env() {
    Switches& s = switches();
    const Switches d;
    for (const Field& f : kFields) {
        if (!f.env) continue;
        const char* e = getenv(f.env);
        if (f.i) s.*(f.i) = e ? (int)std::min<long>(f.hi, std::max<long>(f.lo, atol(e))) : d.*(f.i);
        else s.*(f.b) = e != nullptr;
    }
}

bool set_switch(const char* name, long value) {
    if (!name) return false;
    for (const Field& f : kFields) if (!strcmp(f.name, name)) { assign(switches(), f, value); return true; }
    return false;
}

std::string switches_nondefault() {
    const Switches& s = switches();
    const Switches d;
    std::string out;
    for (const Field& f : kFields) {
        const bool same = f.i ? s.*(f.i) == d.*(f.i) : s.*(f.b) == d.*(f.b);
        if (same) continue;
        if (!out.empty()) out += ' ';
        out += f.name;
        if (f.i) out += "=" + std::to_string(s.*(f.i));
    }
    return out;
}

}
```

### waifu2x-tensorrt_amd/csrc/switches.h

```cpp
#pragma once
#include <string>

namespace w2x {

struct Switches {
    int superbatch = 0;
    int groups = 2;
    int render_parts = 3;
    bool no_graph = false;
    bool no_rolling = false;
    bool poison = false;
    bool check_general = false;
    bool roctx = false;
    bool no_fuse = false;
    bool no_fuse_attn = false;
    bool no_se_fold = false;
    bool no_fuse_head = false;
    bool no_fuse_stem = false;
    bool no_fuse_up = false;
    bool no_conv3h_walk = false;
    bool no_pixgemm = false, no_conv3 = false, no_conv3h = false, no_conv48 = false, no_stem = false;
    bool attn_valu = false;
    bool no_dead_skip = false;
};

Switches& switches();
void switches_from_env();
bool set_switch(const char* name, long value);
std::string switches_nondefault();

}
```

Baseline: 4719 MPix/s.

## Write non-overlap tile pixels from fused MLP head; compose only seam bands

The final fused MLP+image-head kernel now writes each tile's exclusively-owned output pixels straight to the 8-bit BGR frame, using a per-slot HeadTile table uploaded with the slot tables. The compose pass is replaced by a seam-only kernel that blends just the overlap bands between tiles. This is meant to remove most of the compose kernel's reads of the fp16 tile slab and its frame writes. In exchange it adds per-slot table uploads, extra graph-key state, a wait on the output buffer before rolling passes, and narrow eligibility conditions (no TTA, scale 4, no dither, plain BGR).

```diff
diff --git a/waifu2x-tensorrt_amd/csrc/engine.cpp b/waifu2x-tensorrt_amd/csrc/engine.cpp
--- a/waifu2x-tensorrt_amd/csrc/engine.cpp
+++ b/waifu2x-tensorrt_amd/csrc/engine.cpp
@@ -239,6 +239,40 @@
             }
         }
         hipAssert(hipMemcpy2DAsync(d_live, live_stride * sizeof(LiveExt), h_live.data(), count * sizeof(LiveExt), count * sizeof(LiveExt), nops, hipMemcpyHostToDevice, on));
+    }
+    bool head_px_load = false, head_px = false;
+    int head_out_rows = 0, head_out_cols = 0;
+    HeadTile* d_head = nullptr; size_t head_cap = 0, head_count = 0;
+    std::vector<HeadTile> h_head;
+    struct HeadPxScope { Impl* im; ~HeadPxScope() { im->head_px = false; } };
+    bool head_px_frame(const TileGrid& grid, const StripPlan& sp) {
+        const int To = plan.Tout;
+        return head_px_load && job.kind == Job::BGR && !job.rs && !job.chain.src && !job.chain.dst && !deep && (int)dither.mode == kDitherNone && edge == kEdgeReplicate &&
+               !check_general && !profiling && sp.first_tile == 0 && sp.tile_count == grid.count && grid.count > 0 &&
+               To % 4 == 0 && grid.outOvX % 4 == 0 && grid.outOvY % 4 == 0 && 2 * grid.outOvX <= To && 2 * grid.outOvY <= To &&
+               grid.outOvX == ((cfg.overlapX != 0 || cfg.overlapY != 0) ? ovx : 0) && grid.outOvY == ((cfg.overlapX != 0 || cfg.overlapY != 0) ? ovy : 0);
+    }
+    void upload_head_tiles(const TileGrid& grid, size_t count, hipStream_t on) {
+        if (!head_px_load || !count) return;
+        ensure(d_head, head_cap, count * sizeof(HeadTile));
+        head_count = count;
+        std::map<std::pair<int, int>, int> tile_at;
+        for (int t = 0; t < grid.count; ++t) tile_at[{grid.in[t].x, grid.in[t].y}] = t;
+        h_head.assign(count, HeadTile{0, 0, 0, 0, 0, 0});
+        const int To = plan.Tout;
+        for (size_t st = 0; st < count; ++st) {
+            const TileSlot& sl = h_slots[st];
+            if (sl.valid != 1 || sl.aug != 0 || grid.ny <= 0) continue;
+            const auto it = tile_at.find({sl.x, sl.y});
+            if (it == tile_at.end()) continue;
+            const int t = it->second, i = t / grid.ny, j = t % grid.ny;
+            const Rect& r = grid.out[t];
+            const int x0 = i > 0 ? grid.outOvX : 0, x1 = std::min(r.w, i < grid.nx - 1 ? To - grid.outOvX : To);
+            const int y0 = j > 0 ? grid.outOvY : 0, y1 = std::min(r.h, j < grid.ny - 1 ? To - grid.outOvY : To);
+            if (x1 <= x0 || y1 <= y0 || r.x < 0 || r.y < 0 || To > 65535) continue;
+            h_head[st] = HeadTile{r.x, r.y, (uint16_t)x0, (uint16_t)x1, (uint16_t)y0, (uint16_t)y1};
+        }
+        hipAssert(hipMemcpyAsync(d_head, h_head.data(), count * sizeof(HeadTile), hipMemcpyHostToDevice, on));
     }
     float *d_rampx = nullptr, *d_rampy = nullptr;
     int ovx = 0, ovy = 0;
@@ -299,10 +333,12 @@
     static constexpr int kChainStages = 4;
     void* d_chain[kChainStages - 1] = {nullptr, nullptr, nullptr}; size_t chain_cap[kChainStages - 1] = {0, 0, 0};
     hipEvent_t ev_chain_done[kChainStages] = {nullptr, nullptr, nullptr, nullptr}, ev_chain_read[kChainStages - 1] = {nullptr, nullptr, nullptr};
-    struct StageTables { TileSlot* d_slots = nullptr; size_t slots_cap = 0; LiveExt* d_live = nullptr; size_t live_cap = 0, live_stride = 0; std::vector<LiveExt> h_live; std::vector<TileSlot> h_slots; };
+    struct StageTables { TileSlot* d_slots = nullptr; size_t slots_cap = 0; LiveExt* d_live = nullptr; size_t live_cap = 0, live_stride = 0; std::vector<LiveExt> h_live; std::vector<TileSlot> h_slots;
+                         HeadTile* d_head = nullptr; size_t head_cap = 0, head_count = 0; std::vector<HeadTile> h_head; };
     StageTables chain_tables[kChainStages];
     void swap_tables(int k) {
         StageTables& t = chain_tables[k];
+        std::swap(d_head, t.d_head); std::swap(head_cap, t.head_cap); std::swap(head_count, t.head_count); h_head.swap(t.h_head);
         std::swap(d_slots, t.d_slots); std::swap(slots_cap, t.slots_cap); std::swap(d_live, t.d_live); std::swap(live_cap, t.live_cap); std::swap(live_stride, t.live_stride);
         h_live.swap(t.h_live); h_slots.swap(t.h_slots);
     }
@@ -362,6 +398,7 @@
         ensure(d_slots, slots_cap, count * sizeof(TileSlot));
         hipAssert(hipMemcpyAsync(d_slots, h_slots.data(), count * sizeof(TileSlot), hipMemcpyHostToDevice, stream));
         upload_live(grid, count, stream);
+        upload_head_tiles(grid, count, stream);
         ensure(d_slab, slab_cap, slab_slots * plan.Tout * plan.Tout * 4 * plan.elt);
     }
     int last_rows = 0, last_cols = 0, last_batches = 0;
@@ -374,7 +411,7 @@
     static constexpr int kPlanarKey = 67;
     static constexpr int kPlanarRgbaKey = 72;
     static constexpr int kChainKey = 80;
-    using GraphKey = std::tuple<const void*, const void*, const void*, const void*, int, int, int, int>;
+    using GraphKey = std::tuple<const void*, const void*, const void*, const void*, int, int, int, int, const void*>;
     struct PassGraphs { hipGraphExec_t g[4] = {nullptr, nullptr, nullptr, nullptr}; int n = 0; };
     std::map<GraphKey, PassGraphs> graphs;
     std::map<GraphKey, int> graph_seen;
@@ -414,7 +451,7 @@
         canvas_cap = 0;
         for (int k = 0; k + 1 < kChainStages; ++k) { if (d_chain[k]) (void)hipFree(d_chain[k]); d_chain[k] = nullptr; chain_cap[k] = 0; if (ev_chain_read[k]) { (void)hipEventDestroy(ev_chain_read[k]); ev_chain_read[k] = nullptr; } }
         for (hipEvent_t& e : ev_chain_done) if (e) { (void)hipEventDestroy(e); e = nullptr; }
-        for (StageTables& t : chain_tables) { if (t.d_slots) (void)hipFree(t.d_slots); if (t.d_live) (void)hipFree(t.d_live); t = StageTables{}; }
+        for (StageTables& t : chain_tables) { if (t.d_slots) (void)hipFree(t.d_slots); if (t.d_live) (void)hipFree(t.d_live); if (t.d_head) (void)hipFree(t.d_head); t = StageTables{}; }
         report_to = nullptr;
         for (void** q : {(void**)&d_bgr, (void**)&d_alpha, (void**)&d_minmax}) if (*q) { (void)hipFree(*q); *q = nullptr; }
         bgr_cap = alpha_cap = 0;
@@ -423,6 +460,8 @@
         for (void** p : {(void**)&d_frame, (void**)&d_out, (void**)&d_frame2, (void**)&d_out2, &d_slab, &d_slab2, (void**)&d_slots, (void**)&d_live, (void**)&d_rampx, (void**)&d_rampy, (void**)&d_blob_in, (void**)&d_blob_out})
             if (*p) { (void)hipFree(*p); *p = nullptr; }
         frame_cap = out_cap = slab_cap = slab2_cap = slots_cap = 0;
+        if (d_head) { (void)hipFree(d_head); d_head = nullptr; }
+        head_cap = head_count = 0; head_px = head_px_load = false;
         live_cap = live_stride = 0; live_cache.clear();
         shard_rows = shard_cols = 0; shard_halo_slots = 0; rolling = false; one_part_stale = false;
         last_rows = last_cols = last_batches = 0;
@@ -588,6 +627,12 @@
             if (ok) launches.push_back(L);
             else for (int i = L.first; i <= L.last; ++i) launches.push_back(make_launch(plan, L_OP, i, i));
         }
+        head_px_load = false;
+        for (const Launch& L : launches) if (L.kind == L_HEAD) {
+            const GemmParams& g = gemm[L.last];
+            head_px_load = !switches().no_head_pixels && plan.elt == 2 && g.has_clip && g.N == 64 && g.out.Hs == plan.Tout && g.out.Ws == plan.Tout &&
+                           4 * g.aW == plan.Tout && L.last == final_op;
+        }
         launch_planes.assign(launches.size(), {{nullptr, nullptr, nullptr, nullptr}});
         for (size_t k = 0; k < launches.size(); ++k) {
             const Launch& L = launches[k]; std::array<void*, 4>& planes = launch_planes[k];
@@ -604,7 +649,7 @@
     uint8_t* group_ptr(const void* full, int grp) const {
         return full ? (uint8_t*)arena_base + arena_group_offset(arena_bytes, ng_now, grp, (size_t)((const uint8_t*)full - (const uint8_t*)arena_base)) : nullptr;
     }
-    void run_network(void* out_override, int live = -1, int grp = -1, hipStream_t s = nullptr, const LiveExt* ext = nullptr) {
+    void run_network(void* out_override, int live = -1, int grp = -1, hipStream_t s = nullptr, const LiveExt* ext = nullptr, const HeadTile* own = nullptr) {
         if (!s) s = stream;
         const int cap = grp < 0 ? plan.B : plan.B / ng_now;
         if (live < 0 || live > cap) live = cap;
@@ -633,6 +678,14 @@
                     p.live = lv(L.last);
                     p.ti_w = g.wt_frag; p.ti_b = g.bias; p.ti_out = g.out.p; p.ti_Hs = g.out.Hs; p.ti_Ws = g.out.Ws; p.ti_Mrows = g.Mrows; p.ti_aW = g.aW;
                     p.ti_clip = g.has_clip; p.ti_lo = g.clip_lo; p.ti_hi = g.clip_hi;
+                    if (own) {
+                        HeadPixels hp;
+                        const size_t pitch = bgr_step(head_out_cols, false), bytes = pitch * head_out_rows;
+                        if (bytes > 0xFFFFFF00u) throw std::runtime_error("head pixels: the frame exceeds 4 GB");
+                        hp.dst = d_out; hp.pitch = (unsigned)pitch; hp.bytes = (unsigned)bytes; hp.tiles = own;
+                        issue([&] { return launch_mlp96q_px(p, hp, s); });
+                        break;
+                    }
                     issue([&] { return launch_mlp(p, s); });
                     break;
                 }
@@ -780,6 +833,7 @@
         if (which == 1) { std::swap(d_slab, d_slab2); std::swap(slab_cap, slab2_cap); }
         rolling = true;
         hipAssert(hipStreamWaitEvent(stream, ev_cmp[which], 0));
+        if (head_px && out_free) hipAssert(hipStreamWaitEvent(stream, out_free, 0));
         run_passes(rows, cols, sp.tile_count, 0, false, 0, true);
         hipAssert(hipEventRecord(ev_g0[which], stream));
         hipStream_t s2 = gstream[0];
@@ -861,7 +915,10 @@
                 gather_tiles(gp, gs);
             };
             const LiveExt* const ext0 = d_live && slots_off + (size_t)(bi + 1) * B <= live_stride ? d_live + slots_off + (size_t)bi * B : nullptr;
-            auto network_group = [&](int grp, hipStream_t gs) { run_network((uint8_t*)slab_out + (size_t)first[grp] * slot_bytes, first[grp + 1] - first[grp], grp, gs, ext0 ? ext0 + first[grp] : nullptr); };
+            if (head_px && (!d_head || slots_off + (size_t)(bi + 1) * B > head_count)) throw std::runtime_error("head pixels: the slot table does not hold the pass");
+            const HeadTile* const own0 = head_px ? d_head + slots_off + (size_t)bi * B : nullptr;
+            head_out_rows = rows * cfg.scaling; head_out_cols = cols * cfg.scaling;
+            auto network_group = [&](int grp, hipStream_t gs) { run_network((uint8_t*)slab_out + (size_t)first[grp] * slot_bytes, first[grp + 1] - first[grp], grp, gs, ext0 ? ext0 + first[grp] : nullptr, own0 ? own0 + first[grp] : nullptr); };
             auto fork = [&] { hipAssert(hipEventRecord(ev_fork, stream)); for (int grp = 1; grp < NG; ++grp) hipAssert(hipStreamWaitEvent(gstream[grp - 1], ev_fork, 0)); };
             auto join = [&] { for (int grp = 1; grp < NG; ++grp) { hipAssert(hipEventRecord(ev_join[grp - 1], gstream[grp - 1])); hipAssert(hipStreamWaitEvent(stream, ev_join[grp - 1], 0)); } };
             auto run_pass = [&] {
@@ -869,7 +926,7 @@
                     stamp_begin(3, 0);
                     gather_tiles(gp0, stream);
                     stamp_end();
-                    run_network(slab_out, live, -1, nullptr, ext0);
+                    run_network(slab_out, live, -1, nullptr, ext0, own0);
                     return;
                 }
                 ng_now = NG;
@@ -885,7 +942,7 @@
             auto run_eager = [&] { if (per_group) { fork(); for (int grp = 0; grp < NG; ++grp) run_group(grp); if (!no_join) join(); } else { if (rolling && gstream[0]) { join(); } run_pass(); } };
             if (!graphable) run_eager();
             else {
-                const GraphKey key{pass_source(), d_slots + slots_off + (size_t)bi * B, slab_out, arena_base, rows, cols, live, sample_format()};
+                const GraphKey key{pass_source(), d_slots + slots_off + (size_t)bi * B, slab_out, arena_base, rows, cols, live, sample_format(), head_px ? (const void*)d_out : nullptr};
                 auto replay = [&](const PassGraphs& pg) {
                     if (pg.n == 1) { if (rolling && gstream[0]) join(); hipAssert(hipGraphLaunch(pg.g[0], stream)); return; }
                     fork();
@@ -926,7 +983,8 @@
         cp.dst = d_out; cp.dst_step = bgr_step(cp.outW, deep); cp.deep = deep ? 1 : 0;
         cp.x0 = x0; cp.x1 = x1; cp.y0 = y0; cp.y1 = y1; cp.first_tile = first_tile;
         stamp_begin(4, 0);
-        hipAssert(launch_compose(cp, on ? on : stream, dither_now()));
+        if (head_px) hipAssert(launch_compose_seams(cp, grid.outOvX, grid.outOvY, on ? on : stream));
+        else hipAssert(launch_compose(cp, on ? on : stream, dither_now()));
         stamp_end();
     }
     ComposeParams compose_base(int rows, int cols, const TileGrid& grid) const {
@@ -1363,6 +1421,8 @@
         call_slots(c.rows, c.cols, c.grid, c.sp);
         if (!replayable()) one_part_stale = false;
         if (c.resized) job_resize(c.rows, c.cols, c.out_rows, c.out_cols, resizeFilter);
+        HeadPxScope head_scope{this};
+        head_px = head_px_frame(c.grid, c.sp);
         if (!single) { last_ms = run_sequence(count, c.rows, c.cols, c.grid, c.sp, up, down) / count; return; }
         up(0, d_frame, stream);
         run_frame(c.rows, c.cols, c.grid, true, c.sp, ev0);
@@ -1699,13 +1759,14 @@
         return false;
     }
     impl->cfg = config;
+    impl->head_px_load = impl->head_px_load && !config.tta && config.scaling == 4;
     int folds[L_ATTN32 + 1] = {};
     for (const Launch& L : impl->launches) ++folds[L.kind];
     W2X_LOG(info, "Loaded \"" + enginePath + "\": " + std::to_string(plan.ops.size()) + " ops, " + std::to_string(plan.B) + " tiles per pass, activation arena " +
                       std::to_string(impl->arena_bytes >> 20) + " MiB" +
                       (folds[L_STEM] ? ", " + std::to_string(folds[L_STEM]) + " stem folded into the launch of the convolution behind it" : "") +
                       (folds[L_UP] ? ", " + std::to_string(folds[L_UP]) + " transposed convolution folded into the launch of the convolution behind it" : "") +
-                      (folds[L_HEAD] ? ", image head folded into the last MLP launch" : "") +
+                      (folds[L_HEAD] ? std::string(", image head folded into the last MLP launch") + (impl->head_px_load ? " (head pixels: it finishes the tiles' own pixels of plain 8-bit frames)" : "") : std::string()) +
                       (folds[L_ATTN32] + folds[L_MLP32] ? ", " + std::to_string(folds[L_ATTN32]) + " attention and " + std::to_string(folds[L_MLP32]) + " MLP branches as fused fp32-row launches." : "."));
     impl->ovx = (int)std::lround(plan.T * config.scaling * config.overlapX);
     impl->ovy = (int)std::lround(plan.T * config.scaling * config.overlapY);
@@ -1749,6 +1810,8 @@
     impl->deep = bps == 2;
     const StripPlan& sp = c.sp;
     if (sp.tile_count == 0) return true;
+    Impl::HeadPxScope head_scope{&*impl};
+    impl->head_px = parts == 1 && impl->head_px_frame(c.grid, sp);
     const RenderParts rp = render_parts(c.grid, sp, cols, cols * s, rows * s, plan.T, plan.Tout, impl->cfg.tta ? 8 : 1, plan.userB, plan.B,
                                         parts == 1 && !c.resized ? impl->pipeline_parts : 1);
     hipAssert(hipMemcpy2DAsync(impl->d_frame, (size_t)cols * 3 * bps, src.data, src.step, (size_t)rp.x_split * 3 * bps, rows, hipMemcpyHostToDevice, stream));
@@ -2608,6 +2671,8 @@
     DeviceGuard guard(impl->device);
     hipStream_t stream = impl->stream;
     impl->one_part_slots();
+    Impl::HeadPxScope head_scope{&*impl};
+    impl->head_px = impl->head_px_frame(impl->last_grid, impl->last_strip);
     const bool roll = iters > 1 && impl->can_roll(impl->last_strip.tile_count);
     if (roll) impl->ensure(impl->d_slab2, impl->slab2_cap, impl->slab_cap);
     hipAssert(hipEventRecord(impl->ev0, stream));
diff --git a/waifu2x-tensorrt_amd/csrc/k_mlp96q.hip b/waifu2x-tensorrt_amd/csrc/k_mlp96q.hip
--- a/waifu2x-tensorrt_amd/csrc/k_mlp96q.hip
+++ b/waifu2x-tensorrt_amd/csrc/k_mlp96q.hip
@@ -1,4 +1,5 @@
 #include "transformer_device.h"
+#include "prepost_device.h"
 
 #include <algorithm>
 
@@ -41,8 +42,13 @@
 static_assert(RW * PPR % 64 == 0, "flat piece count");
 static_assert(SMEM96Q <= 160 * 1024, "LDS budget");
 
-template <bool TOIMG>
-__global__ __launch_bounds__(NTHR, 3) void mlp96q_kernel(const MlpParams p, int ntiles) {
+__device__ __forceinline__ HeadPixels head_pixels_of() { return HeadPixels(); }
+__device__ __forceinline__ const HeadPixels& head_pixels_of(const HeadPixels& h) { return h; }
+template <bool TOIMG, typename... H>
+__global__ __launch_bounds__(NTHR, 3) void mlp96q_kernel(const MlpParams p, int ntiles, const H... hps) {
+    constexpr bool PX = sizeof...(H) == 1;
+    static_assert(sizeof...(H) <= 1 && (TOIMG || !PX), "finished pixels are the image head's");
+    const HeadPixels& hp = head_pixels_of(hps...);
     extern __shared__ __attribute__((aligned(16))) unsigned char smem[];
     const int tid = threadIdx.x, lane = tid & 63;
     const int wv = __builtin_amdgcn_readfirstlane(tid >> 6);
@@ -216,11 +222,15 @@
 #endif
         W2X_PHASE_FENCE();
         half8 wfh[2][3];
+        const __amdgpu_buffer_rsrc_t WB = make_rsrc(PX ? p.ti_w : nullptr, PX ? 12u * 1024u : 0u);
         if (TOIMG) {
 #pragma unroll
             for (int t = 0; t < 2; ++t)
 #pragma unroll
-                for (int ks = 0; ks < 3; ++ks) wfh[t][ks] = *(const half8*)((const _Float16*)p.ti_w + lane * 8 + (size_t)(t * 3 + ks) * 512);
+                for (int ks = 0; ks < 3; ++ks) {
+                    if constexpr (PX) wfh[t][ks] = __builtin_bit_cast(half8, __builtin_amdgcn_raw_buffer_load_b128(WB, lane * 16u, (unsigned)(t * 3 + ks) * 1024u, 0));
+                    else wfh[t][ks] = *(const half8*)((const _Float16*)p.ti_w + lane * 8 + (size_t)(t * 3 + ks) * 512);
+                }
             W2X_RING_FENCE();
         }
         half8 xres[NP];
@@ -252,6 +262,9 @@
             const int bimg = row0i / p.ti_Mrows, ml0 = row0i - bimg * p.ti_Mrows;
             const int oy0 = ml0 / p.ti_aW, ox0 = ml0 - oy0 * p.ti_aW;
             _Float16* __restrict__ Og = (_Float16*)p.ti_out + (size_t)bimg * p.ti_Hs * p.ti_Ws * 4;
+            HeadTile ht = {};
+            if constexpr (PX) ht = hp.tiles[bimg];
+            const __amdgpu_buffer_rsrc_t FB = make_rsrc(PX ? hp.dst : nullptr, PX ? hp.bytes : 0u);
             const half2v lo2 = {(_Float16)p.ti_lo, (_Float16)p.ti_lo}, hi2 = {(_Float16)p.ti_hi, (_Float16)p.ti_hi};
 #pragma unroll
             for (int th = 0; th < 2; ++th) {
@@ -259,7 +272,10 @@
 #pragma unroll
                 for (int t = 0; t < 2; ++t)
 #pragma unroll
-                    for (int ks = 0; ks < 3; ++ks) wf[t][ks] = th == 0 ? wfh[t][ks] : *(const half8*)(Wt + (size_t)((2 + t) * 3 + ks) * 512);
+                    for (int ks = 0; ks < 3; ++ks) {
+                        if constexpr (PX) wf[t][ks] = th == 0 ? wfh[t][ks] : __builtin_bit_cast(half8, __builtin_amdgcn_raw_buffer_load_b128(WB, lane * 16u, (unsigned)((2 + t) * 3 + ks) * 1024u, 0));
+                        else wf[t][ks] = th == 0 ? wfh[t][ks] : *(const half8*)(Wt + (size_t)((2 + t) * 3 + ks) * 512);
+                    }
                 float4v acc[2][2];
 #pragma unroll
                 for (int t = 0; t < 2; ++t) {
@@ -280,6 +296,8 @@
                     int ox = ox0 + tt * 16 + fr16, oy = oy0;
                     if (ox >= p.ti_aW) { ox -= p.ti_aW; ++oy; }
                     const bool ok = row0 + tt * 16 + fr16 < p.M;
+                    const bool own = PX && ok && 4 * ox >= (int)ht.x0 && 4 * ox + 4 <= (int)ht.x1 && 4 * oy >= (int)ht.y0 && 4 * oy + 4 <= (int)ht.y1;
+                    const unsigned fo = own && g4 < 3 ? (unsigned)(ht.oy + oy * 4) * hp.pitch + (unsigned)(ht.ox + ox * 4) * 3u + g4 * 4u : 0xFFFFFFF0u;
 #pragma unroll
                     for (int t = 0; t < 2; ++t) {
                         half2v v01 = {(_Float16)acc[t][tt][0], (_Float16)acc[t][tt][1]}, v23 = {(_Float16)acc[t][tt][2], (_Float16)acc[t][tt][3]};
@@ -288,7 +306,13 @@
                             asm("v_pk_max_f16 %0, %1, %2\n\tv_pk_min_f16 %0, %0, %3" : "=&v"(v23) : "v"(v23), "v"(lo2), "v"(hi2));
                         }
                         const half4 px = {v01[0], v01[1], v23[0], v23[1]};
-                        if (ok) *(half4*)(Og + ((size_t)(oy * 4 + 2 * th + t) * p.ti_Ws + ox * 4 + g4) * 4) = px;
+                        if constexpr (PX) {
+                            const unsigned q = quantize_bgr((float)px[0], (float)px[1], (float)px[2]);
+                            const unsigned qn = (unsigned)__builtin_amdgcn_ds_bpermute(((lane + 16) & 63) * 4, (int)q);
+                            const unsigned dw = q >> (8 * g4) | qn << (24 - 8 * g4);
+                            __builtin_amdgcn_raw_buffer_store_b32(dw, FB, fo, (unsigned)(2 * th + t) * hp.pitch, 0);
+                        }
+                        if (ok && !own) *(half4*)(Og + ((size_t)(oy * 4 + 2 * th + t) * p.ti_Ws + ox * 4 + g4) * 4) = px;
                     }
                 }
             }
@@ -314,15 +338,16 @@
 #undef W2X_FETCH
 }
 
+
 }
 
 bool mlp96q_supported(const MlpParams& p) { return p.C == C && p.w1_frag && p.w2_frag && p.frag32 && (!p.ti_w || (p.ti_b && p.ti_out && !p.stats_out && p.ti_Mrows > 0 && p.ti_Mrows % RW == 0 && p.ti_aW >= RW && p.M < 0x7FFFFFFFl &&
                                                                  (!p.ti_clip || ((float)(_Float16)p.ti_lo == p.ti_lo && (float)(_Float16)p.ti_hi == p.ti_hi)))); }
 
-hipError_t launch_mlp96q(const MlpParams& p, hipStream_t s) {
+static hipError_t launch_mlp96q_as(const MlpParams& p, const HeadPixels* hp, hipStream_t s) {
     static unsigned lds_ok = 0;
-    static unsigned lds_ok_t = 0;
-    if (hipError_t e = p.ti_w ? ensure_dynamic_lds((const void*)mlp96q_kernel<true>, SMEM96Q, lds_ok_t) : ensure_dynamic_lds((const void*)mlp96q_kernel<false>, SMEM96Q, lds_ok); e != hipSuccess) return e;
+    static unsigned lds_ok_t = 0, lds_ok_px = 0;
+    if (hipError_t e = hp ? ensure_dynamic_lds((const void*)mlp96q_kernel<true, HeadPixels>, SMEM96Q, lds_ok_px) : p.ti_w ? ensure_dynamic_lds((const void*)mlp96q_kernel<true>, SMEM96Q, lds_ok_t) : ensure_dynamic_lds((const void*)mlp96q_kernel<false>, SMEM96Q, lds_ok); e != hipSuccess) return e;
     static int cus[32] = {0};
     int dev = 0;
     if (hipError_t e = hipGetDevice(&dev); e != hipSuccess) return e;
@@ -336,10 +361,17 @@
         const long ntiles = (q.M + RW - 1) / RW;
         const int grid = (int)std::min<long>((ntiles + NWV - 1) / NWV, ncu);
         if ((ntiles + (long)grid * NWV) * (long)(RW * C * 2) > 0xFFFFFFFFl) return hipErrorInvalidValue;
-        if (p.ti_w) hipLaunchKernelGGL(mlp96q_kernel<true>, dim3(grid), dim3(NTHR), SMEM96Q, s, q, (int)ntiles);
+        if (hp) hipLaunchKernelGGL((mlp96q_kernel<true, HeadPixels>), dim3(grid), dim3(NTHR), SMEM96Q, s, q, (int)ntiles, *hp);
+        else if (p.ti_w) hipLaunchKernelGGL(mlp96q_kernel<true>, dim3(grid), dim3(NTHR), SMEM96Q, s, q, (int)ntiles);
         else hipLaunchKernelGGL(mlp96q_kernel<false>, dim3(grid), dim3(NTHR), SMEM96Q, s, q, (int)ntiles);
         return hipGetLastError();
     });
 }
-
-}
+hipError_t launch_mlp96q(const MlpParams& p, hipStream_t s) { return launch_mlp96q_as(p, nullptr, s); }
+bool mlp96q_px_supported(const MlpParams& p, const HeadPixels& hp) { return p.ti_w && mlp96q_supported(p) && p.ti_clip && hp.dst && hp.tiles && hp.pitch > 0 && hp.pitch % 4 == 0 && ((size_t)hp.dst & 3) == 0 && hp.bytes >= hp.pitch && hp.bytes <= 0xFFFFFF00u; }
+hipError_t launch_mlp96q_px(const MlpParams& p, const HeadPixels& hp, hipStream_t s) {
+    if (!mlp96q_px_supported(p, hp)) return hipErrorInvalidValue;
+    return launch_mlp96q_as(p, &hp, s);
+}
+
+}
diff --git a/waifu2x-tensorrt_amd/csrc/k_prepost.hip b/waifu2x-tensorrt_amd/csrc/k_prepost.hip
--- a/waifu2x-tensorrt_amd/csrc/k_prepost.hip
+++ b/waifu2x-tensorrt_amd/csrc/k_prepost.hip
@@ -47,24 +47,16 @@
 
 typedef _Float16 half8 __attribute__((ext_vector_type(8)));
 
-template <typename P, int M = kDitherNone, typename... D>
-__global__ __launch_bounds__(kComposeThreads) void compose_kernel(const ComposeParams p, const D... dzs) {
-    static_assert(dither_pack_ok<M, D...>, "kDitherNone: no argument; else one DitherArgs");
-    const DitherArgs& dz = dither_of(dzs...);
+template <typename P, int M>
+__device__ __forceinline__ void compose_group(const ComposeParams& p, const DitherArgs& dz, int X, int x1, int Y0, int Y1) {
     constexpr bool kHalf = sizeof(P) == 8;
-    const int x1 = p.x1 > 0 ? p.x1 : p.outW, sw = x1 - p.x0;
-    const int gw = (sw + 3) >> 2;
-    const int xg = blockIdx.x * kComposeThreads + threadIdx.x;
-    if (xg >= gw) return;
     const P* tiles = (const P*)p.tiles;
     const int To = p.To, n = To - 1;
-    const int X = p.x0 + 4 * xg;
     const int np = min(4, x1 - X);
     int a0 = X - To + 1; a0 = a0 <= 0 ? 0 : (a0 + p.stride_x - 1) / p.stride_x;
     int b0 = X + 3 - To + 1; b0 = b0 <= 0 ? 0 : (b0 + p.stride_x - 1) / p.stride_x;
     const int a1 = min(p.nx - 1, X / p.stride_x), b1 = min(p.nx - 1, (X + 3) / p.stride_x);
     const bool fast_col = kHalf && np == 4 && !p.tta && !p.deep && a0 == b0 && a1 == b1;
-    const int Y0 = p.y0 + blockIdx.y * kComposeRows, Y1 = min(p.y1 > 0 ? p.y1 : p.outH, Y0 + kComposeRows);
     for (int Y = Y0; Y < Y1; ++Y) {
         uint8_t* d = p.dst + (size_t)Y * p.dst_step + (size_t)X * 3;
         unsigned px[4] = {0u, 0u, 0u, 0u};
@@ -131,6 +123,37 @@
             }
         }
     }
+}
+template <typename P, int M = kDitherNone, typename... D>
+__global__ __launch_bounds__(kComposeThreads) void compose_kernel(const ComposeParams p, const D... dzs) {
+    static_assert(dither_pack_ok<M, D...>, "kDitherNone: no argument; else one DitherArgs");
+    const DitherArgs& dz = dither_of(dzs...);
+    const int x1 = p.x1 > 0 ? p.x1 : p.outW, sw = x1 - p.x0;
+    const int gw = (sw + 3) >> 2;
+    const int xg = blockIdx.x * kComposeThreads + threadIdx.x;
+    if (xg >= gw) return;
+    const int Y0 = p.y0 + blockIdx.y * kComposeRows, Y1 = min(p.y1 > 0 ? p.y1 : p.outH, Y0 + kComposeRows);
+    compose_group<P, M>(p, dz, p.x0 + 4 * xg, x1, Y0, Y1);
+}
+__global__ __launch_bounds__(kComposeThreads) void compose_seams_kernel(const ComposeParams p, int band_x, int band_y, int nrow_a) {
+    const DitherArgs dz = DitherArgs();
+    const int x1 = p.x1 > 0 ? p.x1 : p.outW, y1 = p.y1 > 0 ? p.y1 : p.outH;
+    const int xg = blockIdx.x * kComposeThreads + threadIdx.x;
+    if ((int)blockIdx.y < nrow_a) {
+        const int gx = band_x >> 2;
+        if (gx <= 0 || xg >= (p.nx - 1) * gx) return;
+        const int band = xg / gx, X = (band + 1) * p.stride_x + 4 * (xg - band * gx);
+        if (X < p.x0 || X >= x1) return;
+        const int Y0 = p.y0 + blockIdx.y * kComposeRows;
+        compose_group<half4, kDitherNone>(p, dz, X, x1, Y0, min(y1, Y0 + kComposeRows));
+        return;
+    }
+    const int rb = (band_y + kComposeRows - 1) / kComposeRows, by = blockIdx.y - nrow_a;
+    const int band = by / rb, Yb = (band + 1) * p.stride_y, Y0 = Yb + (by - band * rb) * kComposeRows;
+    const int Ya = max(Y0, p.y0), Yz = min(min(y1, Yb + band_y), Y0 + kComposeRows);
+    const int X = p.x0 + 4 * xg;
+    if (Ya >= Yz || X >= x1) return;
+    compose_group<half4, kDitherNone>(p, dz, X, x1, Ya, Yz);
 }
 
 template <typename P, typename... L>
@@ -590,6 +613,20 @@
     else hipLaunchKernelGGL(compose_kernel<half4>, grid, dim3(kComposeThreads), 0, s, p);
     return hipGetLastError();
 }
+hipError_t launch_compose_seams(const ComposeParams& p, int band_x, int band_y, hipStream_t s) {
+    if (p.fp32 || p.deep || p.tta || p.first_tile != 0 || p.nx < 1 || p.ny < 1 || p.stride_x <= 0 || p.stride_y <= 0 || band_x < 0 || band_y < 0 ||
+        (band_x | p.stride_x | p.x0) % 4 != 0 || band_x > p.stride_x || band_y > p.stride_y) return hipErrorInvalidValue;
+    const int w = (p.x1 > 0 ? p.x1 : p.outW) - p.x0, h = (p.y1 > 0 ? p.y1 : p.outH) - p.y0;
+    if (w <= 0 || h <= 0) return hipSuccess;
+    const int ga = (p.nx - 1) * (band_x / 4), gb = p.ny > 1 && band_y > 0 ? (w + 3) / 4 : 0;
+    const int nrow_a = ga > 0 ? (h + kComposeRows - 1) / kComposeRows : 0;
+    const int nrow_b = gb > 0 ? (p.ny - 1) * ((band_y + kComposeRows - 1) / kComposeRows) : 0;
+    if (nrow_a + nrow_b == 0) return hipSuccess;
+    if (nrow_a + nrow_b > 65535) return hipErrorInvalidValue;
+    const dim3 grid((unsigned)((std::max(ga, gb) + kComposeThreads - 1) / kComposeThreads), (unsigned)(nrow_a + nrow_b));
+    hipLaunchKernelGGL(compose_seams_kernel, grid, dim3(kComposeThreads), 0, s, p, band_x, band_y, nrow_a);
+    return hipGetLastError();
+}
 hipError_t launch_compose_canvas(const ComposeParams& p, float* canvas, hipStream_t s, const LightArgs& l) {
     const int w = (p.x1 > 0 ? p.x1 : p.outW) - p.x0, h = (p.y1 > 0 ? p.y1 : p.outH) - p.y0;
     if (w <= 0 || h <= 0) return hipSuccess;
diff --git a/waifu2x-tensorrt_amd/csrc/kernels.h b/waifu2x-tensorrt_amd/csrc/kernels.h
--- a/waifu2x-tensorrt_amd/csrc/kernels.h
+++ b/waifu2x-tensorrt_amd/csrc/kernels.h
@@ -120,6 +120,16 @@
     const LiveExt* live = nullptr; int live_W = 0, live_H = 0;
     long live_row0 = 0;
 };
+
+struct HeadTile { int ox, oy; uint16_t x0, x1, y0, y1; };
+struct HeadPixels {
+    uint8_t* dst = nullptr; unsigned pitch = 0, bytes = 0;
+    const HeadTile* tiles = nullptr;
+};
+bool mlp96q_px_supported(const MlpParams& p, const HeadPixels& hp);
+hipError_t launch_mlp96q_px(const MlpParams& p, const HeadPixels& hp, hipStream_t s);
+struct ComposeParams;
+hipError_t launch_compose_seams(const ComposeParams& p, int band_x, int band_y, hipStream_t s);
 
 struct SwinAttnParams {
     const void* x = nullptr; void* y = nullptr;
diff --git a/waifu2x-tensorrt_amd/csrc/support.cpp b/waifu2x-tensorrt_amd/csrc/support.cpp
--- a/waifu2x-tensorrt_amd/csrc/support.cpp
+++ b/waifu2x-tensorrt_amd/csrc/support.cpp
@@ -39,6 +39,7 @@
     {"no_fuse_attn", nullptr, &Switches::no_fuse_attn, nullptr, 0, 1},
     {"no_se_fold", nullptr, &Switches::no_se_fold, nullptr, 0, 1},
     {"no_fuse_head", nullptr, &Switches::no_fuse_head, nullptr, 0, 1},
+    {"no_head_pixels", nullptr, &Switches::no_head_pixels, nullptr, 0, 1},
     {"no_fuse_stem", nullptr, &Switches::no_fuse_stem, nullptr, 0, 1},
     {"no_fuse_up", nullptr, &Switches::no_fuse_up, nullptr, 0, 1},
     {"no_conv3h_walk", nullptr, &Switches::no_conv3h_walk, nullptr, 0, 1},
diff --git a/waifu2x-tensorrt_amd/csrc/switches.h b/waifu2x-tensorrt_amd/csrc/switches.h
--- a/waifu2x-tensorrt_amd/csrc/switches.h
+++ b/waifu2x-tensorrt_amd/csrc/switches.h
@@ -16,6 +16,7 @@
     bool no_fuse_attn = false;
     bool no_se_fold = false;
     bool no_fuse_head = false;
+    bool no_head_pixels = false;
     bool no_fuse_stem = false;
     bool no_fuse_up = false;
     bool no_conv3h_walk = false;
```

Measured after the change: 4752 MPix/s (median of 6 runs). About the same (+0.7%).
